# C-H-Chien/Trifocal_Pose_Estimation_using_Improved_GPUHC

Measured on NVIDIA B200. Metric: RANSAC hypotheses/s (312 HC paths each), higher is better.
Workload: dtype c64

## Files before the change

trifocal_pose_estimation_using_improved_gpuhc_b200/codegen/gen_eval.py:

```python
#!/usr/bin/env python3
import os
import sys

import numpy as np

HERE = os.path.dirname(os.path.abspath(__file__))
PKG = os.path.dirname(HERE)
sys.path.insert(0, os.path.dirname(PKG))

N = 30
P_PAD = 33
X_PAD = 30
WARP = 32
SPEC = dict(name="trifocal_2op1p_30x30", n_vars=30, n_params=33, n_tracks=312, hx_terms=8, hx_parts=5, ht_terms=16, ht_parts=6,
            n_depths=8, trifocal=1)


def configure(spec):
    global N, P_PAD, X_PAD, SPEC
    SPEC = dict(spec)
    N, P_PAD, X_PAD = SPEC["n_vars"], SPEC["n_params"], SPEC["n_vars"]
    assert 1 <= N <= 31 and SPEC["hx_parts"] == 5 and SPEC["ht_parts"] == 6


def read_problem_dir(path):
    cfg = {}
    for line in open(os.path.join(path, "gpuhc_settings.yaml")):
        line = line.split("#")[0]
        if ":" in line:
            k, v = line.split(":", 1)
            cfg[k.strip()] = v.strip().strip('"')
    spec = dict(name=cfg["problem_name"], n_vars=int(cfg["Num_Of_Vars"]), n_params=int(cfg["Num_Of_Params"]), n_tracks=int(cfg["Num_Of_Tracks"]),
                hx_terms=int(cfg["dHdx_Max_Terms"]), hx_parts=int(cfg["dHdx_Max_Parts"]), ht_terms=int(cfg["dHdt_Max_Terms"]),
                ht_parts=int(cfg["dHdt_Max_Parts"]), n_depths=int(cfg.get("Num_Of_Depth_Vars", 0)), trifocal=int(cfg["problem_name"] == "trifocal_2op1p_30x30"))
    if spec["trifocal"]:
        spec["n_depths"] = 8
    hx = np.array(open(os.path.join(path, "dHdx_indx.txt")).read().split(), dtype=np.int64)
    ht = np.array(open(os.path.join(path, "dHdt_indx.txt")).read().split(), dtype=np.int64)
    return spec, hx, ht


_TABLES = None


def load_tables():
    if _TABLES is None:
        from trifocal_pose_estimation_using_improved_gpuhc_b200 import fixtures
        prob = fixtures.load_problem()
        hx_flat, ht_flat = prob["dHdx_indx"], prob["dHdt_indx"]
    else:
        hx_flat, ht_flat = _TABLES
    hx = np.asarray(hx_flat).reshape(N, SPEC["hx_terms"], SPEC["hx_parts"], N)
    ht = np.asarray(ht_flat).reshape(SPEC["ht_terms"], SPEC["ht_parts"], N)
    return hx, ht


def parse_terms(hx, ht):
    hx_terms = {}
    for col in range(N):
        for row in range(N):
            lst = []
            for t in range(hx.shape[1]):
                c, a, b, d, e = (int(v) for v in hx[col, t, :, row])
                if c == 0:
                    continue
                xs = [v for v in (d, e) if v != X_PAD]
                assert not (a == P_PAD and b != P_PAD)
                lst.append((c, a, b, xs))
            if lst:
                hx_terms[(row, col)] = lst
    h_terms = {}
    for row in range(N):
        lst = []
        for t in range(ht.shape[0]):
            c, a, b, d, e, f = (int(v) for v in ht[t, :, row])
            if c == 0:
                continue
            xs = [v for v in (d, e, f) if v != X_PAD]
            assert not (a == P_PAD and b != P_PAD)
            lst.append((c, a, b, xs))
        h_terms[row] = lst
    return hx_terms, h_terms


def level_schedule(hx_terms, K1, segments, seg_cols):
    P = np.zeros((N, N), bool)
    for (r, c) in hx_terms:
        P[r, c] = True
    level_of_col = {}
    groups = []
    for g, (seg, cols) in enumerate(zip(segments, seg_cols)):
        busy = {r: -1 for r in seg}
        for c in cols:
            part = [r for r in seg if P[r, c]]
            lvl = 1 + max(busy[r] for r in part)
            u = np.zeros(N, bool)
            for r in part:
                u |= P[r]
            for r in part:
                P[r] |= u
                busy[r] = lvl
            level_of_col[c] = lvl
            groups.append((lvl, g, c, part, u.copy()))
    n_levels = 1 + max([l for l, *_ in groups] or [-1])
    levels, first_shared = [], []
    for T in range(n_levels):
        here = [(g, c, part) for (l, g, c, part, u) in groups if l == T]
        for g in range(len(segments)):
            rows = [r for (gg, c, part) in here if gg == g for r in part]
            assert len(rows) == len(set(rows))
        need = np.zeros(N, bool)
        for (l, g, c, part, u) in groups:
            if l == T:
                need |= u
        shared = [c for c in range(K1, N) if need[c]]
        levels.append(here)
        first_shared.append(min(shared) if shared else N)
    return levels, level_of_col, first_shared


def column_classes(hx_terms):
    rows_of = {c: {r for (r, cc) in hx_terms if cc == c} for c in range(N)}
    order = sorted(range(N), key=lambda c: (-max((len(hx_terms[(r, c)]) for r in rows_of[c]), default=0), c))
    classes = []
    for c in order:
        if not rows_of[c]:
            continue
        for cl in classes:
            if all(not (rows_of[c] & rows_of[o]) for o in cl):
                cl.append(c)
                break
        else:
            classes.append([c])
    return [sorted(cl) for cl in classes]


def schedule(seqs):
    n = max(len(q) for q in seqs)
    return [[q[k] if k < len(q) else None for q in seqs] for k in range(n)]


def analyze_blocks(hx_terms):
    try:
        return _analyze_blocks(hx_terms)
    except AssertionError:
        return 0, [], []


def _analyze_blocks(hx_terms):
    P = np.zeros((N, N), bool)
    for (r, c) in hx_terms:
        P[r, c] = True
    parent = list(range(N))

    def find(a):
        while parent[a] != a:
            parent[a] = parent[parent[a]]
            a = parent[a]
        return a

    cand_of = []
    K1 = N
    for k in range(N):
        cand = [r for r in range(N) if P[r, k]]
        if len(cand) > 6:
            K1 = k
            break
        cand_of.append(cand)
        u = np.zeros(N, bool)
        for r in cand:
            u |= P[r]
        u[:k + 1] = False
        for r in cand:
            P[r] |= u
        for r in cand[1:]:
            parent[find(r)] = find(cand[0])
    comps = {}
    for r in range(N):
        comps.setdefault(find(r), []).append(r)
    assert K1 > 0 and all(len(rows) <= 6 for rows in comps.values())
    comps = sorted(comps.values(), key=lambda rows: min([k for k in range(K1) if set(cand_of[k]) & set(rows)] or [N]))
    segments = []
    for rows in comps:
        for seg in segments:
            if len(seg) + len(rows) <= 6 and len(seg) < 6 and len(rows) < 6:
                seg.extend(rows)
                break
        else:
            segments.append(list(rows))
    segments = [sorted(seg) for seg in segments]
    assert all(len(seg) <= 6 for seg in segments) and len(segments) * 6 <= WARP and sum(len(x) for x in segments) == N
    seg_cols = []
    for seg in segments:
        cols = [k for k in range(K1) if set(cand_of[k]) <= set(seg) and cand_of[k]]
        seg_cols.append(cols)
    assert sorted(c for cols in seg_cols for c in cols) == list(range(K1))
    for g, seg in enumerate(segments):
        for r in seg:
            for c in range(K1):
                assert (not P[r, c]) or c in seg_cols[g], (r, c)
    return K1, segments, seg_cols


def optimise_layout(n_pos, movable_sets, groups, seed=1):
    import random
    rnd = random.Random(seed)
    pos = list(range(n_pos))
    member = {}
    for gi, grp in enumerate(groups):
        for e in grp:
            member.setdefault(e, []).append(gi)

    def gcost(gi):
        cnt = {}
        for e in groups[gi]:
            k = pos[e] % 16
            cnt[k] = cnt.get(k, 0) + 1
        return max(cnt.values())

    cost = [gcost(gi) for gi in range(len(groups))]
    for mv in movable_sets:
        mv = list(mv)
        for sweep in range(8):
            improved = False
            rnd.shuffle(mv)
            for i in range(len(mv)):
                for j in range(i + 1, len(mv)):
                    e, f = mv[i], mv[j]
                    affected = set(member.get(e, [])) | set(member.get(f, []))
                    if not affected:
                        continue
                    before = sum(cost[gi] for gi in affected)
                    pos[e], pos[f] = pos[f], pos[e]
                    after = {gi: gcost(gi) for gi in affected}
                    if sum(after.values()) < before:
                        for gi, c in after.items():
                            cost[gi] = c
                        improved = True
                    else:
                        pos[e], pos[f] = pos[f], pos[e]
            if not improved:
                break
    return pos, sum(cost)


def _groups(slot_rows, field, pad_entry):
    out = []
    for row in slot_rows:
        for half in (range(0, 16), range(16, 32)):
            out.append({pad_entry if row[l] is None else row[l][field] for l in half})
    return out


def build():
    hx, ht = load_tables()
    hx_terms, h_terms = parse_terms(hx, ht)

    cq_keys = set()
    for lst in hx_terms.values():
        cq_keys.update((c, a, b) for c, a, b, _ in lst)
    for lst in h_terms.values():
        cq_keys.update((c, a, b) for c, a, b, _ in lst)
    cq_list = [(0, P_PAD, P_PAD)] + sorted(cq_keys, key=lambda k: (k[2] == P_PAD, k[1], k[2], k[0]))
    cq_index = {k: i for i, k in enumerate(cq_list)}
    dq_keys = set()
    for lst in h_terms.values():
        dq_keys.update((c, a, b) for c, a, b, _ in lst if not (a == P_PAD and b == P_PAD))
    dq_list = [(0, P_PAD, P_PAD)] + sorted(dq_keys, key=lambda k: (k[2] == P_PAD, k[1], k[2], k[0]))
    dq_index = {k: i for i, k in enumerate(dq_list)}

    K1, segments, seg_cols = analyze_blocks(hx_terms)
    levels, level_of_col, sp_first_shared = level_schedule(hx_terms, K1, segments, seg_cols)
    if len(levels) > 4 or (len(levels) + N - K1) % 2:
        K1, segments, seg_cols = 0, [], []
        levels, level_of_col, sp_first_shared = level_schedule(hx_terms, K1, segments, seg_cols)
    SEG = 6
    row_of_lane = [-1] * WARP
    for g, seg in enumerate(segments):
        for i, r in enumerate(seg):
            row_of_lane[g * SEG + i] = r
    if not segments:
        for r in range(N):
            row_of_lane[r] = r
    lane_of_row = [row_of_lane.index(r) for r in range(N)]
    nsp = len(levels)
    nd = N - K1
    col_at = [[None] * nsp for _ in range(WARP)]
    grp_mask = [[0] * nsp for _ in range(WARP)]
    grp_sub = [[0] * nsp for _ in range(WARP)]
    max_sub = 1
    for T, here in enumerate(levels):
        n_in_seg = {}
        for (g, c, part) in here:
            sub = n_in_seg.get(g, 0)
            n_in_seg[g] = sub + 1
            max_sub = max(max_sub, sub + 1)
            mask = 0
            for r in part:
                mask |= 1 << (lane_of_row[r] - g * SEG)
            for r in part:
                ln = lane_of_row[r]
                col_at[ln][T], grp_mask[ln][T], grp_sub[ln][T] = c, mask, sub
    assert max_sub <= 2

    def slot_of(lane, col):
        if col >= K1:
            return nsp + (col - K1)
        assert col_at[lane][level_of_col[col]] == col
        return level_of_col[col]

    pairs, triples = set(), set()
    for lst in list(hx_terms.values()) + list(h_terms.values()):
        for c, a, b, xs in lst:
            if len(xs) == 2:
                pairs.add(tuple(xs))
            elif len(xs) == 3:
                triples.add(tuple(xs))
    pairs, triples = sorted(pairs), sorted(triples)
    XP_PAIR0 = 32
    XP_TRI0 = XP_PAIR0 + ((len(pairs) + WARP - 1) // WARP) * WARP
    XP_TOTAL = XP_TRI0 + ((len(triples) + 7) // 8) * 8

    def xp_index(xs):
        if len(xs) == 0:
            return X_PAD
        if len(xs) == 1:
            return xs[0]
        if len(xs) == 2:
            return XP_PAIR0 + pairs.index(tuple(xs))
        return XP_TRI0 + triples.index(tuple(xs))

    classes = column_classes(hx_terms)
    col_class = {c: ci for ci, cl in enumerate(classes) for c in cl}
    hx_slots = []
    for ci, cl in enumerate(classes):
        seqs = []
        for lane in range(WARP):
            seq = []
            row = row_of_lane[lane]
            if row >= 0:
                cols = [c for c in cl if (row, c) in hx_terms]
                assert len(cols) <= 1
                if cols:
                    for c, a, b, xs in hx_terms[(row, cols[0])]:
                        seq.append((cq_index[(c, a, b)], xp_index(xs)))
            seqs.append(seq)
        for row in schedule(seqs):
            hx_slots.append((ci, row))

    def sched_rows(terms_of_row, index, drop_const):
        seqs = []
        for lane in range(WARP):
            seq = []
            if row_of_lane[lane] >= 0:
                for c, a, b, xs in terms_of_row[row_of_lane[lane]]:
                    if drop_const and a == P_PAD and b == P_PAD:
                        continue
                    seq.append((index[(c, a, b)], xp_index(xs)))
            seqs.append(seq)
        return schedule(seqs)

    h_slots = sched_rows(h_terms, cq_index, False)
    ht_slots = sched_rows(h_terms, dq_index, True)
    while len(ht_slots) < len(h_slots):
        ht_slots.append([None] * WARP)
    assert (nsp + nd) % 2 == 0, "the kernel moves register slots in pairs: levels + dense columns must be even"
    assert all(row_of_lane[l] >= 0 for l in range(N)) and all(row_of_lane[l] < 0 for l in range(N, WARP)), "rows must occupy lanes 0..N-1"
    assert all(-2 <= c <= 5 for lst in list(hx_terms.values()) + list(h_terms.values()) for c, _, _, _ in lst), "coefficients are packed into 3 bits"

    hx_rows = [row for _, row in hx_slots]
    cost0 = [sum(max(sum(1 for e in grp if e % 16 == k) for k in range(16)) for grp in _groups(r, f, pe))
             for r, f, pe in ((hx_rows + h_slots, 0, 0), (ht_slots, 0, 0), (hx_rows + h_slots + ht_slots, 1, X_PAD))]
    cq_pos, c_cq = optimise_layout(len(cq_list), [range(1, len(cq_list))], _groups(hx_rows + h_slots, 0, 0))
    dq_pos, c_dq = optimise_layout(len(dq_list), [range(1, len(dq_list))], _groups(ht_slots, 0, 0))
    xp_pos, c_xp = optimise_layout(XP_TOTAL, [range(XP_PAIR0, XP_TRI0), range(XP_TRI0, XP_TOTAL)],
                                   _groups(hx_rows + h_slots + ht_slots, 1, X_PAD))
    layout_cost = dict(before=cost0, after=[c_cq, c_dq, c_xp])

    def remap(rows, cpos):
        return [[None if p is None else (cpos[p[0]], xp_pos[p[1]]) for p in row] for row in rows]

    hx_slots = [(ci, r) for (ci, _), r in zip(hx_slots, remap(hx_rows, cq_pos))]
    h_slots = remap(h_slots, cq_pos)
    ht_slots = remap(ht_slots, dq_pos)
    cq_by_pos = [(0, P_PAD, P_PAD)] * len(cq_list)
    for e, q in enumerate(cq_pos):
        cq_by_pos[q] = cq_list[e]
    dq_by_pos = [(0, P_PAD, P_PAD)] * len(dq_list)
    for e, q in enumerate(dq_pos):
        dq_by_pos[q] = dq_list[e]
    cq_list, dq_list = cq_by_pos, dq_by_pos
    pair_by_pos = [None] * (XP_TRI0 - XP_PAIR0)
    for i, pr in enumerate(pairs):
        pair_by_pos[xp_pos[XP_PAIR0 + i] - XP_PAIR0] = pr
    tri_by_pos = [None] * (XP_TOTAL - XP_TRI0)
    for i, tr in enumerate(triples):
        tri_by_pos[xp_pos[XP_TRI0 + i] - XP_TRI0] = tr

    nslot = nsp + nd
    scatter = []
    sel_of_lane = [0] * WARP
    nz_of_lane = [0] * WARP
    n_sel = 0
    for t in range(nslot):
        cls_per_lane = []
        for lane in range(WARP):
            col = col_at[lane][t] if t < nsp else (K1 + (t - nsp) if row_of_lane[lane] >= 0 else None)
            cls_per_lane.append(col_class.get(col) if col is not None else None)
        used = sorted({c for c in cls_per_lane if c is not None})
        assert 1 <= len(used) <= 2
        if len(used) == 1:
            scatter.append((used[0], -1, -1))
        else:
            scatter.append((used[0], used[1], n_sel))
            for lane in range(WARP):
                if cls_per_lane[lane] == used[1]:
                    sel_of_lane[lane] |= 1 << n_sel
            n_sel += 1
    for lane in range(WARP):
        row = row_of_lane[lane]
        if row < 0:
            continue
        for c in range(N):
            if (row, c) in hx_terms:
                nz_of_lane[lane] |= 1 << slot_of(lane, c)
    return dict(hx_terms=hx_terms, h_terms=h_terms, cq_list=cq_list, dq_list=dq_list, classes=classes,
                col_class=col_class, hx_slots=hx_slots, h_slots=h_slots, ht_slots=ht_slots,
                K1=K1, segments=segments, seg_cols=seg_cols, row_of_lane=row_of_lane, lane_of_row=lane_of_row,
                nsp=nsp, nd=nd, nslot=nslot, sp_first_shared=sp_first_shared, levels=levels, level_of_col=level_of_col,
                col_at=col_at, grp_mask=grp_mask, grp_sub=grp_sub, max_sub=max_sub, scatter=scatter, sel_of_lane=sel_of_lane, nz_of_lane=nz_of_lane, n_sel=n_sel,
                pairs=pair_by_pos, triples=tri_by_pos, XP_PAIR0=XP_PAIR0, XP_TRI0=XP_TRI0, XP_TOTAL=XP_TOTAL,
                layout_cost=layout_cost)


def pack_word(payload):
    idx, xp = (0, X_PAD) if payload is None else payload
    return (idx * 8) | ((xp * 8) << 16)


def pack_xp_word(xs):
    xs = list(xs) + [X_PAD] * (3 - len(xs))
    return (xs[0] * 8) | ((xs[1] * 8) << 8) | ((xs[2] * 8) << 16)


def pack_build_word(key):
    c, a, b = key
    return (a * 8) | ((b * 8) << 9) | ((c + 2) << 18)


def emit(g, path):
    ncq, ndq = len(g["cq_list"]), len(g["dq_list"])
    rounds = lambda n: (n + WARP - 1) // WARP
    L = []
    w = L.append
    w("// GENERATED by codegen/gen_eval.py from the problem's evaluation-index tables — do not edit.")
    w("// Problem: %s (%d equations, %d unknowns, %d parameters, %d paths)." % (SPEC["name"], N, N, SPEC["n_params"], SPEC["n_tracks"]))
    w("#ifndef HC_PROBLEM_GEN_H")
    w("#define HC_PROBLEM_GEN_H")
    w("#define HCG_N %d" % N)
    w("#define HCG_NUM_PARAMS %d" % SPEC["n_params"])
    w("#define HCG_NUM_CQ %d   /* coef*p_a*p_b table (entry 0 == 0) */" % ncq)
    w("#define HCG_NUM_DQ %d   /* coef*(dp_a*p_b + dp_b*p_a) table (entry 0 == 0) */" % ndq)
    w("#define HCG_CQ_ROUNDS %d" % rounds(ncq))
    w("#define HCG_DQ_ROUNDS %d" % rounds(ndq))
    w("#define HCG_NUM_CLASSES %d" % len(g["classes"]))
    w("#define HCG_HX_SLOTS %d" % len(g["hx_slots"]))
    w("#define HCG_H_SLOTS %d" % len(g["h_slots"]))
    w("#define HCG_HT_SLOTS %d" % len(g["ht_slots"]))
    nnz = len(g["hx_terms"])
    nterms = sum(len(v) for v in g["hx_terms"].values())
    w("#define HCG_HX_NNZ %d" % nnz)
    w("#define HCG_HX_TERMS %d" % nterms)
    w("#define HCG_H_TERMS %d" % sum(len(v) for v in g["h_terms"].values()))
    off_cq = 0
    off_dq = off_cq + rounds(ncq)
    off_pair = off_dq + rounds(ndq)
    off_tri = off_pair + rounds(len(g["pairs"]))
    off_hx = off_tri + rounds(len(g["triples"]))
    w("#define HCG_XP_PAIR0 %d   /* x-product array: [0,32) x itself, then %d pairs, then %d triples */" % (g["XP_PAIR0"], len(g["pairs"]), len(g["triples"])))
    w("#define HCG_XP_TRI0 %d" % g["XP_TRI0"])
    w("#define HCG_XP_TOTAL %d" % g["XP_TOTAL"])
    w("#define HCG_NUM_PAIRS %d" % len(g["pairs"]))
    w("#define HCG_NUM_TRIPLES %d" % len(g["triples"]))
    w("#define HCG_PAIR_ROUNDS %d" % rounds(len(g["pairs"])))
    w("#define HCG_TRI_ROUNDS %d" % rounds(len(g["triples"])))
    w("#define HCG_TBL_PAIR %d" % off_pair)
    w("#define HCG_TBL_TRI %d" % off_tri)
    off_h = off_hx + len(g["hx_slots"])
    off_ht = off_h + len(g["h_slots"])
    total = off_ht + len(g["ht_slots"])
    w("#define HCG_TBL_CQ %d" % off_cq)
    w("#define HCG_TBL_DQ %d" % off_dq)
    w("#define HCG_TBL_HX %d" % off_hx)
    w("#define HCG_TBL_H %d" % off_h)
    w("#define HCG_TBL_HT %d" % off_ht)
    w("#define HCG_TBL_ROWS %d" % total)
    rows = []
    for lst, n in ((g["cq_list"], ncq), (g["dq_list"], ndq)):
        for r in range(rounds(n)):
            rows.append([pack_build_word(lst[r * WARP + l]) if r * WARP + l < n else pack_build_word((0, P_PAD, P_PAD))
                         for l in range(WARP)])
    for lst in (g["pairs"], g["triples"]):
        for r in range(rounds(len(lst))):
            rows.append([pack_xp_word(lst[r * WARP + l]) if r * WARP + l < len(lst) and lst[r * WARP + l] is not None else pack_xp_word([])
                         for l in range(WARP)])
    for _, row in g["hx_slots"]:
        rows.append([pack_word(p) for p in row])
    for row in g["h_slots"]:
        rows.append([pack_word(p) for p in row])
    for row in g["ht_slots"]:
        rows.append([pack_word(p) for p in row])
    assert len(rows) == total
    w("// packed per-lane operand words, [row][lane]")
    w("#define HCG_TBL_INIT { \\")
    for r in rows:
        w("  " + ",".join("0x%08xu" % v for v in r) + ", \\")
    w("}")
    w("// block structure: %d segments of 6 lanes; sparse pivot columns per segment %s; dense columns %d..%d"
      % (len(g["segments"]), g["seg_cols"], g["K1"], N - 1))
    for T, here in enumerate(g["levels"]):
        w("//   level %d: %s" % (T, "  ".join("col %d rows %s" % (c, part) for (_, c, part) in here)))
    w("#define HCG_K1 %d        /* first dense pivot column */" % g["K1"])
    w("#define HCG_NSP %d        /* sparse slots == levels (super-steps) */" % g["nsp"])
    w("#define HCG_ND %d        /* dense slots */" % g["nd"])
    w("#define HCG_NSLOT %d     /* register slots per row */" % g["nslot"])
    w("#define HCG_SEG 6")
    w("#define HCG_NSEG %d" % max(1, len(g["segments"])))
    w("// per super-step: first register slot of the shared columns that can be non-zero in a participating row")
    w("#define HCG_SP_FIRST_SHARED_SLOT_INIT { " + ",".join([str(g["nsp"] + c - g["K1"]) for c in g["sp_first_shared"]] or ["0"]) + " }")
    w("#define HCG_ROW_OF_LANE_INIT { " + ",".join(str(r) for r in g["row_of_lane"]) + " }")
    w("#define HCG_LANE_OF_ROW_INIT { " + ",".join(str(r) for r in g["lane_of_row"]) + " }")
    info, cols, grps = [], [], []
    for lane in range(WARP):
        assert g["nslot"] <= 20 and g["n_sel"] <= 4 and g["nsp"] <= 4
        info.append(g["nz_of_lane"][lane] | (g["sel_of_lane"][lane] << 20))
        packed, gp = 0, 0
        for t in range(g["nsp"]):
            if g["col_at"][lane][t] is not None:
                packed |= g["col_at"][lane][t] << (5 * t)
                gp |= (g["grp_mask"][lane][t] | (g["grp_sub"][lane][t] << 6)) << (7 * t)
        cols.append(packed)
        grps.append(gp)
    w("#define HCG_LANEINFO_INIT { " + ",".join("0x%08xu" % v for v in info) + " }")
    w("#define HCG_LANECOLS_INIT { " + ",".join("0x%08xu" % v for v in cols) + " }   /* 5 bits per level: the private column the lane's row meets there */")
    w("#define HCG_LANEGRP_INIT { " + ",".join("0x%08xu" % v for v in grps) + " }   /* 7 bits per level: lanes of my pivot group (6, relative to the segment) | group index << 6; 0 = idle */")
    w("#define HCG_MAX_GROUPS_PER_SEG %d" % g["max_sub"])
    w("// X(slot, class): one Hx term slot; acc[class] += cq * xprod")
    begs, prev = [], None
    for i, (ci, _) in enumerate(g["hx_slots"]):
        if ci != prev:
            assert prev is None or ci == prev + 1
            begs.append(i)
            prev = ci
    begs.append(len(g["hx_slots"]))
    assert len(begs) == len(g["classes"]) + 1
    w("#define HCG_HX_CLASS_BEGIN_INIT { " + ",".join(str(b) for b in begs) + " }   /* first Hx slot of every class, then the end */")
    w("#define HCG_HX_SLOT_LIST(X) \\")
    for s, (ci, _) in enumerate(g["hx_slots"]):
        w("  X(%d, %d) \\" % (s, ci))
    w("")
    w("// X(slot, classA, classB, selbit): A[slot] = lane has a non-zero there ? acc[selbit set ? classB : classA] : 0")
    w("#define HCG_HX_SCATTER_LIST(X) \\")
    for t, (ca, cb, sb) in enumerate(g["scatter"]):
        w("  X(%d, %d, %d, %d) \\" % (t, ca, cb, sb))
    w("")
    w("// problem identity: the kernel takes every size from this header (codegen/gen_eval.py --problem-dir compiles another problem)")
    w("#define HCG_PROBLEM_NAME \"%s\"" % SPEC["name"])
    w("#define HCG_TRACKS %d        /* homotopy paths per hypothesis (Num_Of_Tracks) */" % SPEC["n_tracks"])
    w("#define HCG_NUM_DEPTHS %d      /* leading variables that are depths: positive-depth pruning tests them (0: no pruning) */" % SPEC["n_depths"])
    w("#define HCG_TRIFOCAL %d        /* 1: the trifocal relative-pose problem (in-kernel scoring, pose records, target-parameter gather) */" % SPEC["trifocal"])
    w("")
    w("#endif")
    text = "\n".join(L) + "\n"
    with open(path, "w") as f:
        f.write(text)
    return text


def compile_problem(problem_dir, out):
    global _TABLES
    spec, hx, ht = read_problem_dir(problem_dir)
    configure(spec)
    _TABLES = (hx, ht)
    g = build()
    emit(g, out)
    return g


def main():
    import argparse
    ap = argparse.ArgumentParser(description=__doc__.split("\n")[0])
    ap.add_argument("--problem-dir", default=None, help="problems/<name>/ in the reference's layout (default: the packaged trifocal_2op1p_30x30 tables)")
    ap.add_argument("--out", default=None, help="header to write (default: csrc/hc_problem_gen.h, or csrc/hc_problem_gen_<name>.h with --problem-dir)")
    a = ap.parse_args()
    if a.problem_dir:
        spec = read_problem_dir(a.problem_dir)[0]
        out = a.out or os.path.join(PKG, "csrc", "hc_problem_gen_%s.h" % spec["name"])
        g = compile_problem(a.problem_dir, out)
        print("problem %s: N %d, parameters %d, paths %d | K1 %d segments %s | classes %s | Hx slots %d, H slots %d, Ht slots %d | cq %d dq %d | pairs %d triples %d"
              % (SPEC["name"], N, SPEC["n_params"], SPEC["n_tracks"], g["K1"], g["segments"], g["classes"], len(g["hx_slots"]), len(g["h_slots"]),
                 len(g["ht_slots"]), len(g["cq_list"]), len(g["dq_list"]), sum(p is not None for p in g["pairs"]), sum(t is not None for t in g["triples"])))
        print("wrote", out)
        return
    g = build()
    out = a.out or os.path.join(PKG, "csrc", "hc_problem_gen.h")
    emit(g, out)
    print("classes:", g["classes"])
    print("K1 %d segments %s seg_cols %s" % (g["K1"], g["segments"], g["seg_cols"]))
    print("row_of_lane", g["row_of_lane"])
    print("scatter", g["scatter"])
    print("cq entries %d, dq entries %d" % (len(g["cq_list"]), len(g["dq_list"])))
    print("Hx slots %d (ref 240), H slots %d (ref 16), Ht slots %d (ref 16)" %
          (len(g["hx_slots"]), len(g["h_slots"]), len(g["ht_slots"])))
    print("gather wavefront model (cq, dq, xp) before/after layout optimisation:", g["layout_cost"])
    print("hx_slots", [(ci, sum(p is not None for p in row)) for ci, row in g["hx_slots"]])
    print("h_slots", [sum(p is not None for p in row) for row in g["h_slots"]])
    print("ht_slots", [sum(p is not None for p in row) for row in g["ht_slots"]])
    print("wrote", out)


if __name__ == "__main__":
    main()
```

trifocal_pose_estimation_using_improved_gpuhc_b200/csrc/hc_problem_gen.h:

```cpp
#ifndef HC_PROBLEM_GEN_H
#define HC_PROBLEM_GEN_H
#define HCG_N 30
#define HCG_NUM_PARAMS 33
#define HCG_NUM_CQ 93
#define HCG_NUM_DQ 89
#define HCG_CQ_ROUNDS 3
#define HCG_DQ_ROUNDS 3
#define HCG_NUM_CLASSES 6
#define HCG_HX_SLOTS 25
#define HCG_H_SLOTS 16
#define HCG_HT_SLOTS 16
#define HCG_HX_NNZ 170
#define HCG_HX_TERMS 558
#define HCG_H_TERMS 360
#define HCG_XP_PAIR0 32
#define HCG_XP_TRI0 96
#define HCG_XP_TOTAL 144
#define HCG_NUM_PAIRS 64
#define HCG_NUM_TRIPLES 48
#define HCG_PAIR_ROUNDS 2
#define HCG_TRI_ROUNDS 2
#define HCG_TBL_PAIR 6
#define HCG_TBL_TRI 8
#define HCG_TBL_CQ 0
#define HCG_TBL_DQ 3
#define HCG_TBL_HX 10
#define HCG_TBL_H 35
#define HCG_TBL_HT 51
#define HCG_TBL_ROWS 67
#define HCG_TBL_INIT { \
  0x000a1108u,0x0001e000u,0x000e1068u,0x00021060u,0x0011e000u,0x00121098u,0x001210c8u,0x000df000u,0x0011f000u,0x0001e008u,0x00121108u,0x000210f8u,0x0011e008u,0x0001f008u,0x0005f008u,0x000df008u,0x000e10e8u,0x00061068u,0x00060030u,0x000e0030u,0x000e1108u,0x00020038u,0x00060038u,0x00021030u,0x00120038u,0x000e1010u,0x000e1018u,0x000e1020u,0x000e1028u,0x000610c8u,0x00061030u,0x000e1030u, \
  0x00121030u,0x000e10d8u,0x001210c0u,0x000e1038u,0x00121038u,0x000e1040u,0x000e1048u,0x000e1050u,0x000e1058u,0x0011f008u,0x00061060u,0x000e1060u,0x00121060u,0x00021068u,0x000e10c8u,0x000e1080u,0x00121068u,0x000e1070u,0x000e1078u,0x00021100u,0x000e10b8u,0x000e0038u,0x00061090u,0x000e1090u,0x00121090u,0x00021098u,0x0001f000u,0x000e1098u,0x00061108u,0x000e10a0u,0x000e10a8u,0x000e10b0u, \
  0x0005f000u,0x00120030u,0x000610c0u,0x000e10c0u,0x00061038u,0x0005e008u,0x000de000u,0x00021090u,0x000610f0u,0x000e10d0u,0x00021038u,0x000e10e0u,0x000210c0u,0x000210f0u,0x00020030u,0x000e10f0u,0x0005e000u,0x000de008u,0x000610f8u,0x000e10f8u,0x001210f8u,0x001210f0u,0x00061100u,0x000e1100u,0x00121100u,0x00021108u,0x000210c8u,0x00061098u,0x000e1088u,0x000a1108u,0x000a1108u,0x000a1108u, \
  0x000a1108u,0x0001e000u,0x0005e000u,0x000de000u,0x0011e000u,0x00060038u,0x0005f000u,0x000df000u,0x0011f000u,0x0001e008u,0x0005e008u,0x000de008u,0x0011e008u,0x0001f008u,0x0005f008u,0x000df008u,0x00061068u,0x0011f008u,0x00060030u,0x000e0030u,0x000e10c8u,0x00020038u,0x00021090u,0x000e0038u,0x00120038u,0x000e1010u,0x000e1018u,0x000e1020u,0x000e1028u,0x00021030u,0x00061030u,0x000e1030u, \
  0x00121030u,0x00021038u,0x00061038u,0x000e1038u,0x00121038u,0x000e1040u,0x000e1048u,0x000e1050u,0x000e1058u,0x00021060u,0x00061060u,0x000e1060u,0x00121060u,0x00021068u,0x00020030u,0x000e1068u,0x00121068u,0x000e1070u,0x000e1078u,0x000e1080u,0x000e1088u,0x00120030u,0x00061090u,0x000e1090u,0x00121090u,0x00021098u,0x00061098u,0x000e1098u,0x00121098u,0x000e10a0u,0x000e10a8u,0x000e10b0u, \
  0x000e10b8u,0x000210c0u,0x000610c0u,0x000e10c0u,0x00061100u,0x000210c8u,0x000610c8u,0x0001f000u,0x001210c8u,0x000e10d0u,0x000e10d8u,0x000e10e0u,0x000e10e8u,0x000210f0u,0x000610f0u,0x000e10f0u,0x001210f0u,0x000210f8u,0x000610f8u,0x000e10f8u,0x001210f8u,0x00021100u,0x001210c0u,0x000e1100u,0x00121100u,0x000a1108u,0x000a1108u,0x000a1108u,0x000a1108u,0x000a1108u,0x000a1108u,0x000a1108u, \
  0x00f0f0f0u,0x00f0f0f0u,0x00f0d000u,0x00f0d800u,0x00f0e000u,0x00f0d808u,0x00f0c008u,0x00f0c808u,0x00f0c078u,0x00f0c860u,0x00f0e008u,0x00f0e808u,0x00f0d008u,0x00f0f0f0u,0x00f0f0f0u,0x00f0d860u,0x00f0f0f0u,0x00f0e860u,0x00f0d060u,0x00f0c878u,0x00f0d078u,0x00f0d878u,0x00f0c060u,0x00f0e878u,0x00f0c0c0u,0x00f0c8c0u,0x00f0d0c0u,0x00f0f0f0u,0x00f0d0c8u,0x00f0d0d0u,0x00f0f0f0u,0x00f0e0d8u, \
  0x00f0e8d8u,0x00f0d8d8u,0x00f0e8e0u,0x00f0e8e8u,0x00f0f0f0u,0x00f0f0f0u,0x00f0e0e0u,0x00f0f0f0u,0x00f0f0f0u,0x00f0e800u,0x00f0f0f0u,0x00f0f0f0u,0x00f0f0f0u,0x00f0c800u,0x00f0f0f0u,0x00f0c000u,0x00f0f0f0u,0x00f0f0f0u,0x00f0f0f0u,0x00f0f0f0u,0x00f0c8c8u,0x00f0f0f0u,0x00f0f0f0u,0x00f0f0f0u,0x00f0f0f0u,0x00f0f0f0u,0x00f0f0f0u,0x00f0e078u,0x00f0e060u,0x00f0f0f0u,0x00f0f0f0u,0x00f0f0f0u, \
  0x00c0c000u,0x00c8c000u,0x00d0c000u,0x00c8c800u,0x00d0c800u,0x00d0d000u,0x00e8e078u,0x00e0d800u,0x00e8d800u,0x00e0e000u,0x00e8e000u,0x00e8e060u,0x00c0c008u,0x00c8c008u,0x00d0c008u,0x00c8c808u,0x00d0c808u,0x00d0d008u,0x00d8d808u,0x00e0d808u,0x00e8d808u,0x00d0c060u,0x00e8e008u,0x00e8e808u,0x00c0c060u,0x00c8c060u,0x00d8d800u,0x00c8c860u,0x00d0c860u,0x00d0d060u,0x00d8d860u,0x00e0d860u, \
  0x00e8d860u,0x00e0e060u,0x00e8e800u,0x00e8e860u,0x00c0c078u,0x00c8c078u,0x00d0c078u,0x00c8c878u,0x00d0c878u,0x00d0d078u,0x00d8d878u,0x00e0d878u,0x00e8d878u,0x00e0e078u,0x00e0e008u,0x00e8e878u,0x00f0f0f0u,0x00f0f0f0u,0x00f0f0f0u,0x00f0f0f0u,0x00f0f0f0u,0x00f0f0f0u,0x00f0f0f0u,0x00f0f0f0u,0x00f0f0f0u,0x00f0f0f0u,0x00f0f0f0u,0x00f0f0f0u,0x00f0f0f0u,0x00f0f0f0u,0x00f0f0f0u,0x00f0f0f0u, \
  0x00d00120u,0x00c00050u,0x00c80100u,0x00e80120u,0x00d80050u,0x00e00100u,0x00d00180u,0x00c00050u,0x00c80160u,0x00e80180u,0x00d80050u,0x00e00160u,0x00f000c8u,0x00f000d0u,0x00f000a0u,0x00f000d8u,0x00f000e0u,0x00f000a0u,0x00d00028u,0x01c001d8u,0x00c801c0u,0x00e80028u,0x020801d8u,0x00e001c0u,0x00d00030u,0x01c00170u,0x00c80110u,0x00e80030u,0x02080170u,0x00e00110u,0x00f00000u,0x00f00000u, \
  0x00c802c8u,0x00f00220u,0x00c00250u,0x00e002c8u,0x00f00220u,0x00d80250u,0x00c802c8u,0x00f00088u,0x00c00168u,0x00e002c8u,0x00f00088u,0x00d80168u,0x00f00000u,0x00f00000u,0x00f00000u,0x00f00000u,0x00f00000u,0x00f00000u,0x00f001b0u,0x00d00238u,0x00c001c8u,0x00f001b0u,0x00e80238u,0x00d801c8u,0x00f00210u,0x00d00260u,0x00c002d0u,0x00f00210u,0x00e80260u,0x00d802d0u,0x00f00000u,0x00f00000u, \
  0x00f000f0u,0x00d000b8u,0x01c000a0u,0x00f000f0u,0x00e800b8u,0x020800a0u,0x00f00150u,0x00d00018u,0x01c000a0u,0x00f00150u,0x00e80018u,0x020800a0u,0x00f00000u,0x00f00000u,0x00f00000u,0x00f00000u,0x00f00000u,0x00f00000u,0x01c001b0u,0x00f002d8u,0x01d00238u,0x020801b0u,0x00f002d8u,0x02000238u,0x01c00210u,0x00f000e8u,0x01d00260u,0x02080210u,0x00f000e8u,0x02000260u,0x00f00000u,0x00f00000u, \
  0x01d002c8u,0x01e002c8u,0x02a000a0u,0x020002c8u,0x021002c8u,0x023000a0u,0x01d002c8u,0x01e002c8u,0x02a000a0u,0x020002c8u,0x021002c8u,0x023000a0u,0x00f00000u,0x00f00000u,0x00f00000u,0x00f00000u,0x00f00000u,0x00f00000u,0x02a001b8u,0x02a002d8u,0x01e001c8u,0x023001b8u,0x023002d8u,0x021001c8u,0x02a00218u,0x02a000e8u,0x01e002d0u,0x02300218u,0x023000e8u,0x021002d0u,0x00f00000u,0x00f00000u, \
  0x01c000f0u,0x01c00118u,0x01e801e0u,0x020800f0u,0x02080118u,0x021801e0u,0x01c00150u,0x01c00010u,0x01e801e0u,0x02080150u,0x02080010u,0x021801e0u,0x00f00000u,0x00f00000u,0x00f00000u,0x00f00000u,0x00f00000u,0x00f00000u,0x01e801b8u,0x01e801d8u,0x00f00000u,0x021801b8u,0x021801d8u,0x00f00000u,0x01e80218u,0x01e80170u,0x00f00000u,0x02180218u,0x02180170u,0x00f00000u,0x00f00000u,0x00f00000u, \
  0x02a000f8u,0x02a00220u,0x01d000b8u,0x023000f8u,0x02300220u,0x020000b8u,0x02a00158u,0x02a00088u,0x01d00018u,0x02300158u,0x02300088u,0x02000018u,0x00f00000u,0x00f00000u,0x00f00000u,0x00f00000u,0x00f00000u,0x00f00000u,0x01c801c8u,0x01c80238u,0x00f00000u,0x01f801c8u,0x01f80238u,0x00f00000u,0x01c802d0u,0x01c80260u,0x00f00000u,0x01f802d0u,0x01f80260u,0x00f00000u,0x00f00000u,0x00f00000u, \
  0x01e800f8u,0x01e80118u,0x01e00250u,0x021800f8u,0x02180118u,0x02100250u,0x01e80158u,0x01e80010u,0x01e00168u,0x02180158u,0x02180010u,0x02100168u,0x00f00000u,0x00f00000u,0x00f00000u,0x00f00000u,0x00f00000u,0x00f00000u,0x00f00000u,0x00f00000u,0x00f00000u,0x00f00000u,0x00f00000u,0x00f00000u,0x00f00000u,0x00f00000u,0x00f00000u,0x00f00000u,0x00f00000u,0x00f00000u,0x00f00000u,0x00f00000u, \
  0x01c80250u,0x01c800b8u,0x00f001e0u,0x01f80250u,0x01f800b8u,0x00f001e0u,0x01c80168u,0x01c80018u,0x00f001e0u,0x01f80168u,0x01f80018u,0x00f001e0u,0x00f00000u,0x00f00000u,0x00f00000u,0x00f00000u,0x00f00000u,0x00f00000u,0x00f00000u,0x00f00000u,0x00f00000u,0x00f00000u,0x00f00000u,0x00f00000u,0x00f00000u,0x00f00000u,0x00f00000u,0x00f00000u,0x00f00000u,0x00f00000u,0x00f00000u,0x00f00000u, \
  0x011002c8u,0x00000050u,0x02780050u,0x024802c8u,0x00000050u,0x01180050u,0x016002c8u,0x00080050u,0x01300050u,0x015802c8u,0x00080050u,0x01280050u,0x00d00268u,0x00f002a8u,0x00c002a8u,0x00e80268u,0x00f002a8u,0x00d802a8u,0x00d00058u,0x00f002a0u,0x00c002a0u,0x00e80058u,0x00f002a0u,0x00d802a0u,0x00d00198u,0x00f002c0u,0x00c002c0u,0x00e80198u,0x00f002c0u,0x00d802c0u,0x00f00000u,0x00f00000u, \
  0x027800b8u,0x026800b8u,0x00000250u,0x011800b8u,0x012000b8u,0x00000250u,0x01300018u,0x01380018u,0x00080168u,0x01280018u,0x01500018u,0x00080168u,0x00c00008u,0x00c80008u,0x00f00048u,0x00d80008u,0x00e00008u,0x00f00048u,0x00c001d0u,0x00c801d0u,0x006001c8u,0x00d801d0u,0x00e001d0u,0x006001c8u,0x00c00270u,0x00c80270u,0x007802d0u,0x00d80270u,0x00e00270u,0x007802d0u,0x00f00000u,0x00f00000u, \
  0x02680250u,0x02780120u,0x011000b8u,0x01200250u,0x01180120u,0x024800b8u,0x01380168u,0x01300180u,0x01600018u,0x01500168u,0x01280180u,0x01580018u,0x00c80048u,0x00c00060u,0x00d00008u,0x00e00048u,0x00d80060u,0x00e80008u,0x00c80068u,0x00c00148u,0x00f00068u,0x00e00068u,0x00d80148u,0x00f00068u,0x00c800a8u,0x00c000c0u,0x00f000a8u,0x00e000a8u,0x00d800c0u,0x00f000a8u,0x00f00000u,0x00f00000u, \
  0x00f00000u,0x00f00000u,0x00f00000u,0x00f00000u,0x00f00000u,0x00f00000u,0x00f00000u,0x00f00000u,0x00f00000u,0x00f00000u,0x00f00000u,0x00f00000u,0x00f00000u,0x00f00000u,0x00f00000u,0x00f00000u,0x00f00000u,0x00f00000u,0x01b00238u,0x01480238u,0x00d001d0u,0x01780238u,0x02e00238u,0x00e801d0u,0x01400260u,0x01980260u,0x00d00270u,0x01a80260u,0x02d80260u,0x00e80270u,0x00f00000u,0x00f00000u, \
  0x00f00000u,0x00f00000u,0x00f00000u,0x00f00000u,0x00f00000u,0x00f00000u,0x00f00000u,0x00f00000u,0x00f00000u,0x00f00000u,0x00f00000u,0x00f00000u,0x00f00000u,0x00f00000u,0x00f00000u,0x00f00000u,0x00f00000u,0x00f00000u,0x014801c8u,0x01b00028u,0x01900238u,0x02e001c8u,0x01780028u,0x01880238u,0x019802d0u,0x01400030u,0x01a00260u,0x02d802d0u,0x01a80030u,0x01b80260u,0x00f00000u,0x00f00000u, \
  0x02680100u,0x011002c8u,0x00000100u,0x01200100u,0x024802c8u,0x00000100u,0x01380160u,0x016002c8u,0x00080160u,0x01500160u,0x015802c8u,0x00080160u,0x00c80020u,0x00d00268u,0x00f00020u,0x00e00020u,0x00e80268u,0x00f00020u,0x00c80040u,0x00d00058u,0x00f00040u,0x00e00040u,0x00e80058u,0x00f00040u,0x00c80208u,0x00d00198u,0x00f00208u,0x00e00208u,0x00e80198u,0x00f00208u,0x00f00000u,0x00f00000u, \
  0x000002c8u,0x027800b8u,0x02680050u,0x000002c8u,0x011800b8u,0x01200050u,0x000802c8u,0x01300018u,0x01380050u,0x000802c8u,0x01280018u,0x01500050u,0x00f00268u,0x00c00008u,0x00c802a8u,0x00f00268u,0x00d80008u,0x00e002a8u,0x00f00058u,0x00c001d0u,0x006001c0u,0x00f00058u,0x00d801d0u,0x006001c0u,0x00f00198u,0x00c00270u,0x00780110u,0x00f00198u,0x00d80270u,0x00780110u,0x00f00000u,0x00f00000u, \
  0x02780250u,0x02680250u,0x01100250u,0x01180250u,0x01200250u,0x02480250u,0x01300168u,0x01380168u,0x01600168u,0x01280168u,0x01500168u,0x01580168u,0x00c00048u,0x00c80048u,0x00d00048u,0x00d80048u,0x00e00048u,0x00e80048u,0x00c00068u,0x00c80068u,0x00c802a0u,0x00d80068u,0x00e00068u,0x00e002a0u,0x00c000a8u,0x00c800a8u,0x00c802c0u,0x00d800a8u,0x00e000a8u,0x00e002c0u,0x00f00000u,0x00f00000u, \
  0x00f00000u,0x00f00000u,0x00f00000u,0x00f00000u,0x00f00000u,0x00f00000u,0x00f00000u,0x00f00000u,0x00f00000u,0x00f00000u,0x00f00000u,0x00f00000u,0x00f00000u,0x00f00000u,0x00f00000u,0x00f00000u,0x00f00000u,0x00f00000u,0x014801c0u,0x01b00238u,0x00d00068u,0x02e001c0u,0x01780238u,0x00e80068u,0x01980110u,0x01400260u,0x00d000a8u,0x02d80110u,0x01a80260u,0x00e800a8u,0x00f00000u,0x00f00000u, \
  0x00f00000u,0x00f00000u,0x00f00000u,0x00f00000u,0x00f00000u,0x00f00000u,0x00f00000u,0x00f00000u,0x00f00000u,0x00f00000u,0x00f00000u,0x00f00000u,0x00f00000u,0x00f00000u,0x00f00000u,0x00f00000u,0x00f00000u,0x00f00000u,0x01b001c8u,0x014801c8u,0x019001c8u,0x017801c8u,0x02e001c8u,0x018801c8u,0x014002d0u,0x019802d0u,0x01a002d0u,0x01a802d0u,0x02d802d0u,0x01b802d0u,0x00f00000u,0x00f00000u, \
  0x00000120u,0x01100120u,0x011002c8u,0x00000120u,0x02480120u,0x024802c8u,0x00080180u,0x01600180u,0x016002c8u,0x00080180u,0x01580180u,0x015802c8u,0x00f00060u,0x00d00060u,0x00d00268u,0x00f00060u,0x00e80060u,0x00e80268u,0x00f00148u,0x00d00148u,0x00d00058u,0x00f00148u,0x00e80148u,0x00e80058u,0x00f000c0u,0x00d000c0u,0x00d00198u,0x00f000c0u,0x00e800c0u,0x00e80198u,0x00f00000u,0x00f00000u, \
  0x027802c8u,0x026802c8u,0x027800b8u,0x011802c8u,0x012002c8u,0x011800b8u,0x013002c8u,0x013802c8u,0x01300018u,0x012802c8u,0x015002c8u,0x01280018u,0x00c00268u,0x00c80268u,0x00c00008u,0x00d80268u,0x00e00268u,0x00d80008u,0x00600028u,0x00600238u,0x00c001d0u,0x00600028u,0x00600238u,0x00d801d0u,0x00780030u,0x00780260u,0x00c00270u,0x00780030u,0x00780260u,0x00d80270u,0x00f00000u,0x00f00000u, \
  0x01100100u,0x000000b8u,0x02680250u,0x02480100u,0x000000b8u,0x01200250u,0x01600160u,0x00080018u,0x01380168u,0x01580160u,0x00080018u,0x01500168u,0x00d00020u,0x00f00008u,0x00c80048u,0x00e80020u,0x00f00008u,0x00e00048u,0x00c00058u,0x00c80058u,0x00c80068u,0x00d80058u,0x00e00058u,0x00e00068u,0x00c00198u,0x00c80198u,0x00c800a8u,0x00d80198u,0x00e00198u,0x00e000a8u,0x00f00000u,0x00f00000u, \
  0x00f00000u,0x00f00000u,0x00f00000u,0x00f00000u,0x00f00000u,0x00f00000u,0x00f00000u,0x00f00000u,0x00f00000u,0x00f00000u,0x00f00000u,0x00f00000u,0x00f00000u,0x00f00000u,0x00f00000u,0x00f00000u,0x00f00000u,0x00f00000u,0x00d00040u,0x00f001d0u,0x01b00238u,0x00e80040u,0x00f001d0u,0x01780238u,0x00d00208u,0x00f00270u,0x01400260u,0x00e80208u,0x00f00270u,0x01a80260u,0x00f00000u,0x00f00000u, \
  0x00f00000u,0x00f00000u,0x00f00000u,0x00f00000u,0x00f00000u,0x00f00000u,0x00f00000u,0x00f00000u,0x00f00000u,0x00f00000u,0x00f00000u,0x00f00000u,0x00f00000u,0x00f00000u,0x00f00000u,0x00f00000u,0x00f00000u,0x00f00000u,0x019001c0u,0x01900028u,0x014801c8u,0x018801c0u,0x01880028u,0x02e001c8u,0x01a00110u,0x01a00030u,0x019802d0u,0x01b80110u,0x01b80030u,0x02d802d0u,0x00f00000u,0x00f00000u, \
  0x00f00128u,0x00f00130u,0x00f000a0u,0x00f00138u,0x00f00140u,0x00f000a0u,0x00f00188u,0x00f00190u,0x00f000a0u,0x00f00178u,0x00f002e0u,0x00f000a0u,0x00f00000u,0x00f00000u,0x00f00000u,0x00f00000u,0x00f00000u,0x00f00000u,0x00f000c8u,0x00f000d0u,0x00f000a0u,0x00f000d8u,0x00f000e0u,0x00f000a0u,0x00f00128u,0x00f00130u,0x00f000a0u,0x00f00138u,0x00f00140u,0x00f000a0u,0x00f00000u,0x00f00000u, \
  0x00f001e0u,0x00f001e0u,0x00f001e0u,0x00f001e0u,0x00f001e0u,0x00f001e0u,0x00f001e0u,0x00f001e0u,0x00f001e0u,0x00f001e0u,0x00f001e0u,0x00f001e0u,0x00f001e0u,0x00f001e0u,0x00f001e0u,0x00f001e0u,0x00f001e0u,0x00f001e0u,0x00f001e8u,0x00f001f0u,0x00f00000u,0x00f001f8u,0x00f001a0u,0x00f00000u,0x00f00248u,0x00f00108u,0x00f00000u,0x00f00258u,0x00f00080u,0x00f00000u,0x00f00000u,0x00f00000u, \
  0x00180128u,0x00180130u,0x001800a0u,0x00300138u,0x00300140u,0x003000a0u,0x00200188u,0x00200190u,0x002000a0u,0x00380178u,0x003802e0u,0x003800a0u,0x001000c8u,0x001000d0u,0x001000a0u,0x002800d8u,0x002800e0u,0x002800a0u,0x004000c8u,0x004000d0u,0x004000a0u,0x004800d8u,0x004800e0u,0x004800a0u,0x00500128u,0x00500130u,0x005000a0u,0x00580138u,0x00580140u,0x005800a0u,0x00f00000u,0x00f00000u, \
  0x000000f0u,0x00000220u,0x000001e0u,0x000000f0u,0x00000220u,0x000001e0u,0x00080150u,0x00080088u,0x000801e0u,0x00080150u,0x00080088u,0x000801e0u,0x00f00280u,0x00f00228u,0x00f00240u,0x00f00280u,0x00f00228u,0x00f00240u,0x00f00200u,0x00f00070u,0x00f00290u,0x00f00200u,0x00f00070u,0x00f00290u,0x00f00090u,0x00f000b0u,0x00f002b0u,0x00f00090u,0x00f000b0u,0x00f002b0u,0x00f00000u,0x00f00000u, \
  0x009001e0u,0x009801e0u,0x00a001e0u,0x00a801e0u,0x00b001e0u,0x00b801e0u,0x009001e0u,0x009801e0u,0x00a001e0u,0x00a801e0u,0x00b001e0u,0x00b801e0u,0x009001e0u,0x009801e0u,0x00a001e0u,0x00a801e0u,0x00b001e0u,0x00b801e0u,0x006001b0u,0x006002d8u,0x01c00298u,0x006001b0u,0x006002d8u,0x02080298u,0x00780210u,0x007800e8u,0x01c002b8u,0x00780210u,0x007800e8u,0x020802b8u,0x00f00000u,0x00f00000u, \
  0x026802c8u,0x02780050u,0x030000a0u,0x012002c8u,0x01180050u,0x03d000a0u,0x013802c8u,0x01300050u,0x036000a0u,0x015002c8u,0x01280050u,0x039000a0u,0x00c80268u,0x00c002a8u,0x01c00278u,0x00e00268u,0x00d802a8u,0x02080278u,0x006801e8u,0x006801f0u,0x02a00298u,0x007001f8u,0x007001a0u,0x02300298u,0x00800248u,0x00800108u,0x02a002b8u,0x00880258u,0x00880080u,0x023002b8u,0x00f00000u,0x00f00000u, \
  0x030000f0u,0x03000118u,0x031800a0u,0x03d000f0u,0x03d00118u,0x034800a0u,0x03600150u,0x03600010u,0x037800a0u,0x03900150u,0x03900010u,0x047000a0u,0x01c00280u,0x01c00288u,0x02a00278u,0x02080280u,0x02080288u,0x02300278u,0x00c80058u,0x00c002a0u,0x01e80290u,0x00e00058u,0x00d802a0u,0x02180290u,0x00c80198u,0x00c002c0u,0x01e802b0u,0x00e00198u,0x00d802c0u,0x021802b0u,0x00f00000u,0x00f00000u, \
  0x031800f8u,0x03180220u,0x032801e0u,0x034800f8u,0x03480220u,0x041001e0u,0x03780158u,0x03780088u,0x038801e0u,0x04700158u,0x04700088u,0x03b801e0u,0x02a00230u,0x02a00228u,0x01e80240u,0x02300230u,0x02300228u,0x02180240u,0x01c00200u,0x01c00078u,0x00c80040u,0x02080200u,0x02080078u,0x00e00040u,0x01c00090u,0x01c001a8u,0x00c80208u,0x02080090u,0x020801a8u,0x00e00208u,0x00f00000u,0x00f00000u, \
  0x032800f8u,0x03280118u,0x02680100u,0x041000f8u,0x04100118u,0x01200100u,0x03880158u,0x03880010u,0x01380160u,0x03b80158u,0x03b80010u,0x01500160u,0x01e80230u,0x01e80288u,0x00c80020u,0x02180230u,0x02180288u,0x00e00020u,0x02a00038u,0x02a00070u,0x00c00068u,0x02300038u,0x02300070u,0x00d80068u,0x02a00098u,0x02a000b0u,0x00c000a8u,0x02300098u,0x023000b0u,0x00d800a8u,0x00f00000u,0x00f00000u, \
  0x01100120u,0x011000b8u,0x02780250u,0x02480120u,0x024800b8u,0x01180250u,0x01600180u,0x01600018u,0x01300168u,0x01580180u,0x01580018u,0x01280168u,0x00d00060u,0x00d00008u,0x00c00048u,0x00e80060u,0x00e80008u,0x00d80048u,0x01e80038u,0x01e80078u,0x014801c0u,0x02180038u,0x02180078u,0x02e001c0u,0x01e80098u,0x01e801a8u,0x01980110u,0x02180098u,0x021801a8u,0x02d80110u,0x00f00000u,0x00f00000u, \
  0x031002c8u,0x032002c8u,0x031000b8u,0x034002c8u,0x035002c8u,0x034000b8u,0x037002c8u,0x038002c8u,0x03700018u,0x03a002c8u,0x03b002c8u,0x03a00018u,0x01d00268u,0x01e00268u,0x01d00008u,0x02000268u,0x02100268u,0x02000008u,0x03c001b0u,0x03c001d8u,0x01b001c8u,0x03f001b0u,0x03f001d8u,0x017801c8u,0x04200210u,0x04200170u,0x014002d0u,0x04500210u,0x04500170u,0x01a802d0u,0x00f00000u,0x00f00000u, \
  0x03080250u,0x030800b8u,0x03200250u,0x03380250u,0x033800b8u,0x03500250u,0x03680168u,0x03680018u,0x03800168u,0x03980168u,0x03980018u,0x03b00168u,0x01c80048u,0x01c80008u,0x01e00048u,0x01f80048u,0x01f80008u,0x02100048u,0x03d801b8u,0x03d802d8u,0x01d001d0u,0x040801b8u,0x040802d8u,0x020001d0u,0x04380218u,0x043800e8u,0x01d00270u,0x04680218u,0x046800e8u,0x02000270u,0x00f00000u,0x00f00000u, \
  0x00f00000u,0x00f00000u,0x00f00000u,0x00f00000u,0x00f00000u,0x00f00000u,0x00f00000u,0x00f00000u,0x00f00000u,0x00f00000u,0x00f00000u,0x00f00000u,0x00f00000u,0x00f00000u,0x00f00000u,0x00f00000u,0x00f00000u,0x00f00000u,0x03e801b8u,0x03e801d8u,0x01e00068u,0x041801b8u,0x041801d8u,0x02100068u,0x04480218u,0x04480170u,0x01e000a8u,0x04780218u,0x04780170u,0x021000a8u,0x00f00000u,0x00f00000u, \
  0x00f00000u,0x00f00000u,0x00f00000u,0x00f00000u,0x00f00000u,0x00f00000u,0x00f00000u,0x00f00000u,0x00f00000u,0x00f00000u,0x00f00000u,0x00f00000u,0x00f00000u,0x00f00000u,0x00f00000u,0x00f00000u,0x00f00000u,0x00f00000u,0x00d00148u,0x00d001d0u,0x03a80238u,0x00e80148u,0x00e801d0u,0x04000238u,0x00d000c0u,0x00d00270u,0x04300260u,0x00e800c0u,0x00e80270u,0x04600260u,0x00f00000u,0x00f00000u, \
  0x00f00000u,0x00f00000u,0x00f00000u,0x00f00000u,0x00f00000u,0x00f00000u,0x00f00000u,0x00f00000u,0x00f00000u,0x00f00000u,0x00f00000u,0x00f00000u,0x00f00000u,0x00f00000u,0x00f00000u,0x00f00000u,0x00f00000u,0x00f00000u,0x01900028u,0x01900238u,0x03e001c8u,0x01880028u,0x01880238u,0x035801c8u,0x01a00030u,0x01a00260u,0x044002d0u,0x01b80030u,0x01b80260u,0x033002d0u,0x00f00000u,0x00f00000u, \
  0x00f00000u,0x00f00000u,0x00f00000u,0x00f00000u,0x00f00000u,0x00f00000u,0x00f00000u,0x00f00000u,0x00f00000u,0x00f00000u,0x00f00000u,0x00f00000u,0x00f00000u,0x00f00000u,0x00f00000u,0x00f00000u,0x00f00000u,0x00f00000u,0x01d00058u,0x01e00058u,0x00f00000u,0x02000058u,0x02100058u,0x00f00000u,0x01d00198u,0x01e00198u,0x00f00000u,0x02000198u,0x02100198u,0x00f00000u,0x00f00000u,0x00f00000u, \
  0x00f00000u,0x00f00000u,0x00f00000u,0x00f00000u,0x00f00000u,0x00f00000u,0x00f00000u,0x00f00000u,0x00f00000u,0x00f00000u,0x00f00000u,0x00f00000u,0x00f00000u,0x00f00000u,0x00f00000u,0x00f00000u,0x00f00000u,0x00f00000u,0x01c80068u,0x01c801d0u,0x00f00000u,0x01f80068u,0x01f801d0u,0x00f00000u,0x01c800a8u,0x01c80270u,0x00f00000u,0x01f800a8u,0x01f80270u,0x00f00000u,0x00f00000u,0x00f00000u, \
  0x00f00000u,0x00f00000u,0x00f00000u,0x00f00000u,0x00f00000u,0x00f00000u,0x00f00000u,0x00f00000u,0x00f00000u,0x00f00000u,0x00f00000u,0x00f00000u,0x00f00000u,0x00f00000u,0x00f00000u,0x00f00000u,0x00f00000u,0x00f00000u,0x03c801c8u,0x03c80238u,0x00f00000u,0x03f801c8u,0x03f80238u,0x00f00000u,0x042802d0u,0x04280260u,0x00f00000u,0x045802d0u,0x04580260u,0x00f00000u,0x00f00000u,0x00f00000u, \
  0x00180128u,0x00180130u,0x02680100u,0x00300138u,0x00300140u,0x01200100u,0x00200188u,0x00200190u,0x01380160u,0x00380198u,0x003801a0u,0x01500160u,0x001000c8u,0x001000d0u,0x00f00270u,0x002800d8u,0x002800e0u,0x00f00270u,0x004000c8u,0x004000d0u,0x00f00290u,0x004800d8u,0x004800e0u,0x00f00290u,0x00500128u,0x00500130u,0x00f00220u,0x00580138u,0x00580140u,0x00f00220u,0x00f00000u,0x00f00000u, \
  0x000000f0u,0x00000110u,0x02780108u,0x000000f0u,0x00000110u,0x01180108u,0x00080150u,0x00080080u,0x01300168u,0x00080150u,0x00080080u,0x01280168u,0x00f00010u,0x00f00050u,0x01c00278u,0x00f00010u,0x00f00050u,0x02080278u,0x00f00030u,0x00f00070u,0x01c00298u,0x00f00030u,0x00f00070u,0x02080298u,0x00f00090u,0x00f00028u,0x01c002b8u,0x00f00090u,0x00f00028u,0x020802b8u,0x00f00000u,0x00f00000u, \
  0x030000f0u,0x03000118u,0x031000e8u,0x03d000f0u,0x03d00118u,0x034000e8u,0x03600150u,0x03600178u,0x03700148u,0x03900150u,0x03900178u,0x03a00148u,0x00c80268u,0x00c00280u,0x02a00278u,0x00e00268u,0x00d80280u,0x02300278u,0x006001b0u,0x006001d0u,0x02a00298u,0x006001b0u,0x006001d0u,0x02300298u,0x00780210u,0x00780230u,0x02a002b8u,0x00780210u,0x00780230u,0x023002b8u,0x00f00000u,0x00f00000u, \
  0x031800f8u,0x03180110u,0x03200108u,0x034800f8u,0x03480110u,0x03500108u,0x03780158u,0x03780080u,0x03800168u,0x04700158u,0x04700080u,0x03b00168u,0x01c00010u,0x01c00058u,0x01e80270u,0x02080010u,0x02080058u,0x02180270u,0x006801e8u,0x006801f0u,0x01e80290u,0x007001f8u,0x00700200u,0x02180290u,0x00800248u,0x00800250u,0x01e80220u,0x00880258u,0x00880260u,0x02180220u,0x00f00000u,0x00f00000u, \
  0x032800f8u,0x03280118u,0x00f00000u,0x041000f8u,0x04100118u,0x00f00000u,0x03880158u,0x03880178u,0x00f00000u,0x03b80158u,0x03b80178u,0x00f00000u,0x02a00018u,0x02a00050u,0x00c80020u,0x02300018u,0x02300050u,0x00e00020u,0x00c80288u,0x00c002a0u,0x00c80040u,0x00e00288u,0x00d802a0u,0x00e00040u,0x00c802a8u,0x00c002c0u,0x00c801a8u,0x00e002a8u,0x00d802c0u,0x00e001a8u,0x00f00000u,0x00f00000u, \
  0x01100120u,0x011000e8u,0x00f00000u,0x02480120u,0x024800e8u,0x00f00000u,0x01600180u,0x01600148u,0x00f00000u,0x01580180u,0x01580148u,0x00f00000u,0x01e80018u,0x01e80058u,0x00c00048u,0x02180018u,0x02180058u,0x00d80048u,0x01c00030u,0x01c00078u,0x00c00068u,0x02080030u,0x02080078u,0x00d80068u,0x01c00090u,0x01c000b8u,0x00c000a8u,0x02080090u,0x020800b8u,0x00d800a8u,0x00f00000u,0x00f00000u, \
  0x03080108u,0x030800e8u,0x00f00000u,0x03380108u,0x033800e8u,0x00f00000u,0x03680168u,0x03680148u,0x00f00000u,0x03980168u,0x03980148u,0x00f00000u,0x00d00060u,0x00d00008u,0x01d00008u,0x00e80060u,0x00e80008u,0x02000008u,0x02a00038u,0x02a00070u,0x014801c0u,0x02300038u,0x02300070u,0x02e001c0u,0x02a00098u,0x02a00028u,0x019802b0u,0x02300098u,0x02300028u,0x02d802b0u,0x00f00000u,0x00f00000u, \
  0x00f00000u,0x00f00000u,0x00f00000u,0x00f00000u,0x00f00000u,0x00f00000u,0x00f00000u,0x00f00000u,0x00f00000u,0x00f00000u,0x00f00000u,0x00f00000u,0x01d00268u,0x01e00268u,0x01e00048u,0x02000268u,0x02100268u,0x02100048u,0x01e80038u,0x01e80078u,0x01b001c8u,0x02180038u,0x02180078u,0x017801c8u,0x01e80098u,0x01e800b8u,0x01400228u,0x02180098u,0x021800b8u,0x01a80228u,0x00f00000u,0x00f00000u, \
  0x00f00000u,0x00f00000u,0x00f00000u,0x00f00000u,0x00f00000u,0x00f00000u,0x00f00000u,0x00f00000u,0x00f00000u,0x00f00000u,0x00f00000u,0x00f00000u,0x01c80048u,0x01c80008u,0x00f00000u,0x01f80048u,0x01f80008u,0x00f00000u,0x03c001b0u,0x03c001d8u,0x01d00238u,0x03f001b0u,0x03f001d8u,0x02000238u,0x04200210u,0x042000a0u,0x01d00170u,0x04500210u,0x045000a0u,0x02000170u,0x00f00000u,0x00f00000u, \
  0x00f00000u,0x00f00000u,0x00f00000u,0x00f00000u,0x00f00000u,0x00f00000u,0x00f00000u,0x00f00000u,0x00f00000u,0x00f00000u,0x00f00000u,0x00f00000u,0x00f00000u,0x00f00000u,0x00f00000u,0x00f00000u,0x00f00000u,0x00f00000u,0x03d801b8u,0x03d801d0u,0x01e00068u,0x040801b8u,0x040801d0u,0x02100068u,0x04380218u,0x04380230u,0x01e000a8u,0x04680218u,0x04680230u,0x021000a8u,0x00f00000u,0x00f00000u, \
  0x00f00000u,0x00f00000u,0x00f00000u,0x00f00000u,0x00f00000u,0x00f00000u,0x00f00000u,0x00f00000u,0x00f00000u,0x00f00000u,0x00f00000u,0x00f00000u,0x00f00000u,0x00f00000u,0x00f00000u,0x00f00000u,0x00f00000u,0x00f00000u,0x03e801b8u,0x03e801d8u,0x03a800b0u,0x041801b8u,0x041801d8u,0x040000b0u,0x04480218u,0x044800a0u,0x04300208u,0x04780218u,0x047800a0u,0x04600208u,0x00f00000u,0x00f00000u, \
  0x00f00000u,0x00f00000u,0x00f00000u,0x00f00000u,0x00f00000u,0x00f00000u,0x00f00000u,0x00f00000u,0x00f00000u,0x00f00000u,0x00f00000u,0x00f00000u,0x00f00000u,0x00f00000u,0x00f00000u,0x00f00000u,0x00f00000u,0x00f00000u,0x00d00088u,0x00d00238u,0x03e001c8u,0x00e80088u,0x00e80238u,0x035801c8u,0x00d000c0u,0x00d00170u,0x04400228u,0x00e800c0u,0x00e80170u,0x03300228u,0x00f00000u,0x00f00000u, \
  0x00f00000u,0x00f00000u,0x00f00000u,0x00f00000u,0x00f00000u,0x00f00000u,0x00f00000u,0x00f00000u,0x00f00000u,0x00f00000u,0x00f00000u,0x00f00000u,0x00f00000u,0x00f00000u,0x00f00000u,0x00f00000u,0x00f00000u,0x00f00000u,0x019001e0u,0x019000b0u,0x00f00000u,0x018801e0u,0x018800b0u,0x00f00000u,0x01a00240u,0x01a00208u,0x00f00000u,0x01b80240u,0x01b80208u,0x00f00000u,0x00f00000u,0x00f00000u, \
  0x00f00000u,0x00f00000u,0x00f00000u,0x00f00000u,0x00f00000u,0x00f00000u,0x00f00000u,0x00f00000u,0x00f00000u,0x00f00000u,0x00f00000u,0x00f00000u,0x00f00000u,0x00f00000u,0x00f00000u,0x00f00000u,0x00f00000u,0x00f00000u,0x01d00288u,0x01e00288u,0x00f00000u,0x02000288u,0x02100288u,0x00f00000u,0x01d002a8u,0x01e002a8u,0x00f00000u,0x020002a8u,0x021002a8u,0x00f00000u,0x00f00000u,0x00f00000u, \
  0x00f00000u,0x00f00000u,0x00f00000u,0x00f00000u,0x00f00000u,0x00f00000u,0x00f00000u,0x00f00000u,0x00f00000u,0x00f00000u,0x00f00000u,0x00f00000u,0x00f00000u,0x00f00000u,0x00f00000u,0x00f00000u,0x00f00000u,0x00f00000u,0x01c80068u,0x01c80238u,0x00f00000u,0x01f80068u,0x01f80238u,0x00f00000u,0x01c800a8u,0x01c80170u,0x00f00000u,0x01f800a8u,0x01f80170u,0x00f00000u,0x00f00000u,0x00f00000u, \
  0x00f00000u,0x00f00000u,0x00f00000u,0x00f00000u,0x00f00000u,0x00f00000u,0x00f00000u,0x00f00000u,0x00f00000u,0x00f00000u,0x00f00000u,0x00f00000u,0x00f00000u,0x00f00000u,0x00f00000u,0x00f00000u,0x00f00000u,0x00f00000u,0x03c801c8u,0x03c800b0u,0x00f00000u,0x03f801c8u,0x03f800b0u,0x00f00000u,0x04280228u,0x04280208u,0x00f00000u,0x04580228u,0x04580208u,0x00f00000u,0x00f00000u,0x00f00000u, \
}
#define HCG_K1 18
#define HCG_NSP 4
#define HCG_ND 12
#define HCG_NSLOT 16
#define HCG_SEG 6
#define HCG_NSEG 5
#define HCG_SP_FIRST_SHARED_SLOT_INIT { 4,4,4,10 }
#define HCG_ROW_OF_LANE_INIT { 3,4,5,12,13,14,6,7,8,15,16,17,0,1,2,9,10,11,18,19,20,24,25,26,21,22,23,27,28,29,-1,-1 }
#define HCG_LANE_OF_ROW_INIT { 12,13,14,0,1,2,6,7,8,15,16,17,3,4,5,9,10,11,18,19,20,24,25,26,21,22,23,27,28,29 }
#define HCG_LANEINFO_INIT { 0x00201c13u,0x00201c23u,0x00201c43u,0x0020e085u,0x0020e105u,0x0020e205u,0x00201c13u,0x00201c23u,0x00201c43u,0x0020e085u,0x0020e105u,0x0020e205u,0x00001c11u,0x00001c21u,0x00001c41u,0x0000e081u,0x0000e101u,0x0000e201u,0x00501c07u,0x00501c07u,0x00501c03u,0x0050e00bu,0x0050e00bu,0x0050e003u,0x00501c07u,0x00501c07u,0x00501c03u,0x0050e00bu,0x0050e00bu,0x0050e003u,0x00000000u,0x00000000u }
#define HCG_LANECOLS_INIT { 0x00001860u,0x00001860u,0x00001860u,0x00001860u,0x00001860u,0x00001860u,0x00001c81u,0x00001c81u,0x00001c81u,0x00001c81u,0x00001c81u,0x00001c81u,0x00000002u,0x00000002u,0x00000002u,0x00000005u,0x00000005u,0x00000005u,0x00073588u,0x00073588u,0x00073588u,0x00073589u,0x00073589u,0x00073589u,0x0008c1eau,0x0008c1eau,0x0008c1eau,0x0008c1ebu,0x0008c1ebu,0x0008c1ebu,0x00000000u,0x00000000u }
#define HCG_LANEGRP_INIT { 0x000fdfbfu,0x000fdfbfu,0x000fdfbfu,0x000fdfbfu,0x000fdfbfu,0x000fdfbfu,0x000fdfbfu,0x000fdfbfu,0x000fdfbfu,0x000fdfbfu,0x000fdfbfu,0x000fdfbfu,0x00000007u,0x00000007u,0x00000007u,0x00000078u,0x00000078u,0x00000078u,0x07efdf87u,0x07efdf87u,0x07efdf87u,0x07efdff8u,0x07efdff8u,0x07efdff8u,0x07efdf87u,0x07efdf87u,0x07efdf87u,0x07efdff8u,0x07efdff8u,0x07efdff8u,0x00000000u,0x00000000u }
#define HCG_MAX_GROUPS_PER_SEG 2
#define HCG_HX_CLASS_BEGIN_INIT { 0,8,13,18,23,24,25 }
#define HCG_HX_SLOT_LIST(X) \
  X(0, 0) \
  X(1, 0) \
  X(2, 0) \
  X(3, 0) \
  X(4, 0) \
  X(5, 0) \
  X(6, 0) \
  X(7, 0) \
  X(8, 1) \
  X(9, 1) \
  X(10, 1) \
  X(11, 1) \
  X(12, 1) \
  X(13, 2) \
  X(14, 2) \
  X(15, 2) \
  X(16, 2) \
  X(17, 2) \
  X(18, 3) \
  X(19, 3) \
  X(20, 3) \
  X(21, 3) \
  X(22, 3) \
  X(23, 4) \
  X(24, 5) \

#define HCG_HX_SCATTER_LIST(X) \
  X(0, 0, 4, 0) \
  X(1, 0, 4, 1) \
  X(2, 4, 5, 2) \
  X(3, 5, -1, -1) \
  X(4, 5, -1, -1) \
  X(5, 5, -1, -1) \
  X(6, 5, -1, -1) \
  X(7, 5, -1, -1) \
  X(8, 5, -1, -1) \
  X(9, 5, -1, -1) \
  X(10, 1, -1, -1) \
  X(11, 2, -1, -1) \
  X(12, 3, -1, -1) \
  X(13, 1, -1, -1) \
  X(14, 2, -1, -1) \
  X(15, 3, -1, -1) \

#define HCG_PROBLEM_NAME "trifocal_2op1p_30x30"
#define HCG_TRACKS 312
#define HCG_NUM_DEPTHS 8
#define HCG_TRIFOCAL 1

#endif
```

trifocal_pose_estimation_using_improved_gpuhc_b200/csrc/hc_problem_gen_coupled_quadrics_8x8.h:

```cpp
#ifndef HC_PROBLEM_GEN_H
#define HC_PROBLEM_GEN_H
#define HCG_N 8
#define HCG_NUM_PARAMS 10
#define HCG_NUM_CQ 14
#define HCG_NUM_DQ 12
#define HCG_CQ_ROUNDS 1
#define HCG_DQ_ROUNDS 1
#define HCG_NUM_CLASSES 7
#define HCG_HX_SLOTS 7
#define HCG_H_SLOTS 5
#define HCG_HT_SLOTS 5
#define HCG_HX_NNZ 38
#define HCG_HX_TERMS 38
#define HCG_H_TERMS 34
#define HCG_XP_PAIR0 32
#define HCG_XP_TRI0 64
#define HCG_XP_TOTAL 72
#define HCG_NUM_PAIRS 32
#define HCG_NUM_TRIPLES 8
#define HCG_PAIR_ROUNDS 1
#define HCG_TRI_ROUNDS 1
#define HCG_TBL_PAIR 2
#define HCG_TBL_TRI 3
#define HCG_TBL_CQ 0
#define HCG_TBL_DQ 1
#define HCG_TBL_HX 4
#define HCG_TBL_H 11
#define HCG_TBL_HT 16
#define HCG_TBL_ROWS 21
#define HCG_TBL_INIT { \
  0x0008a050u,0x00040000u,0x00041008u,0x00042010u,0x00043018u,0x00044020u,0x00045028u,0x00046030u,0x00047038u,0x000c9040u,0x000ca040u,0x000ca048u,0x000ca050u,0x0010a050u,0x0008a050u,0x0008a050u,0x0008a050u,0x0008a050u,0x0008a050u,0x0008a050u,0x0008a050u,0x0008a050u,0x0008a050u,0x0008a050u,0x0008a050u,0x0008a050u,0x0008a050u,0x0008a050u,0x0008a050u,0x0008a050u,0x0008a050u,0x0008a050u, \
  0x0008a050u,0x00040000u,0x00041008u,0x00042010u,0x00043018u,0x00044020u,0x00045028u,0x00046030u,0x00047038u,0x000c9040u,0x000ca040u,0x000ca048u,0x0008a050u,0x0008a050u,0x0008a050u,0x0008a050u,0x0008a050u,0x0008a050u,0x0008a050u,0x0008a050u,0x0008a050u,0x0008a050u,0x0008a050u,0x0008a050u,0x0008a050u,0x0008a050u,0x0008a050u,0x0008a050u,0x0008a050u,0x0008a050u,0x0008a050u,0x0008a050u, \
  0x00400000u,0x00401000u,0x00400808u,0x00404040u,0x00401008u,0x00401010u,0x00401810u,0x00402010u,0x00401818u,0x00402818u,0x00402020u,0x00403020u,0x00402828u,0x00403028u,0x00403828u,0x00400030u,0x00403030u,0x00403830u,0x00400838u,0x00403838u,0x00404040u,0x00404040u,0x00404040u,0x00404040u,0x00404040u,0x00404040u,0x00401808u,0x00404040u,0x00404040u,0x00404040u,0x00404040u,0x00404040u, \
  0x00181008u,0x00383028u,0x00404040u,0x00404040u,0x00404040u,0x00404040u,0x00404040u,0x00404040u,0x00404040u,0x00404040u,0x00404040u,0x00404040u,0x00404040u,0x00404040u,0x00404040u,0x00404040u,0x00404040u,0x00404040u,0x00404040u,0x00404040u,0x00404040u,0x00404040u,0x00404040u,0x00404040u,0x00404040u,0x00404040u,0x00404040u,0x00404040u,0x00404040u,0x00404040u,0x00404040u,0x00404040u, \
  0x00000068u,0x00100050u,0x00200068u,0x00300050u,0x00400058u,0x00100050u,0x00400058u,0x00300050u,0x00400000u,0x00400000u,0x00400000u,0x00400000u,0x00400000u,0x00400000u,0x00400000u,0x00400000u,0x00400000u,0x00400000u,0x00400000u,0x00400000u,0x00400000u,0x00400000u,0x00400000u,0x00400000u,0x00400000u,0x00400000u,0x00400000u,0x00400000u,0x00400000u,0x00400000u,0x00400000u,0x00400000u, \
  0x00180050u,0x00080068u,0x01300048u,0x00400000u,0x00380050u,0x00400058u,0x00400000u,0x00400000u,0x00400000u,0x00400000u,0x00400000u,0x00400000u,0x00400000u,0x00400000u,0x00400000u,0x00400000u,0x00400000u,0x00400000u,0x00400000u,0x00400000u,0x00400000u,0x00400000u,0x00400000u,0x00400000u,0x00400000u,0x00400000u,0x00400000u,0x00400000u,0x00400000u,0x00400000u,0x00400000u,0x00400000u, \
  0x00400058u,0x00200050u,0x01d00048u,0x00400000u,0x00400000u,0x00000050u,0x00100068u,0x00400000u,0x00400000u,0x00400000u,0x00400000u,0x00400000u,0x00400000u,0x00400000u,0x00400000u,0x00400000u,0x00400000u,0x00400000u,0x00400000u,0x00400000u,0x00400000u,0x00400000u,0x00400000u,0x00400000u,0x00400000u,0x00400000u,0x00400000u,0x00400000u,0x00400000u,0x00400000u,0x00400000u,0x00400000u, \
  0x00080050u,0x00400058u,0x01200048u,0x00400000u,0x00400000u,0x00400000u,0x00280050u,0x00180068u,0x00400000u,0x00400000u,0x00400000u,0x00400000u,0x00400000u,0x00400000u,0x00400000u,0x00400000u,0x00400000u,0x00400000u,0x00400000u,0x00400000u,0x00400000u,0x00400000u,0x00400000u,0x00400000u,0x00400000u,0x00400000u,0x00400000u,0x00400000u,0x00400000u,0x00400000u,0x00400000u,0x00400000u, \
  0x01880048u,0x00400000u,0x00380050u,0x00280068u,0x00400000u,0x00400000u,0x00180050u,0x00400058u,0x00400000u,0x00400000u,0x00400000u,0x00400000u,0x00400000u,0x00400000u,0x00400000u,0x00400000u,0x00400000u,0x00400000u,0x00400000u,0x00400000u,0x00400000u,0x00400000u,0x00400000u,0x00400000u,0x00400000u,0x00400000u,0x00400000u,0x00400000u,0x00400000u,0x00400000u,0x00400000u,0x00400000u, \
  0x01700048u,0x00400000u,0x00400058u,0x00000050u,0x00300068u,0x00400000u,0x00400000u,0x00200050u,0x00400000u,0x00400000u,0x00400000u,0x00400000u,0x00400000u,0x00400000u,0x00400000u,0x00400000u,0x00400000u,0x00400000u,0x00400000u,0x00400000u,0x00400000u,0x00400000u,0x00400000u,0x00400000u,0x00400000u,0x00400000u,0x00400000u,0x00400000u,0x00400000u,0x00400000u,0x00400000u,0x00400000u, \
  0x01680048u,0x00400000u,0x00280050u,0x00400058u,0x00080050u,0x00380068u,0x00400000u,0x00400000u,0x00400000u,0x00400000u,0x00400000u,0x00400000u,0x00400000u,0x00400000u,0x00400000u,0x00400000u,0x00400000u,0x00400000u,0x00400000u,0x00400000u,0x00400000u,0x00400000u,0x00400000u,0x00400000u,0x00400000u,0x00400000u,0x00400000u,0x00400000u,0x00400000u,0x00400000u,0x00400000u,0x00400000u, \
  0x01000060u,0x01100060u,0x01500060u,0x01600060u,0x01800060u,0x01980060u,0x01280060u,0x01400060u,0x00400000u,0x00400000u,0x00400000u,0x00400000u,0x00400000u,0x00400000u,0x00400000u,0x00400000u,0x00400000u,0x00400000u,0x00400000u,0x00400000u,0x00400000u,0x00400000u,0x00400000u,0x00400000u,0x00400000u,0x00400000u,0x00400000u,0x00400000u,0x00400000u,0x00400000u,0x00400000u,0x00400000u, \
  0x00400008u,0x00400010u,0x00400028u,0x00400030u,0x00400038u,0x00400040u,0x00400018u,0x00400020u,0x00400000u,0x00400000u,0x00400000u,0x00400000u,0x00400000u,0x00400000u,0x00400000u,0x00400000u,0x00400000u,0x00400000u,0x00400000u,0x00400000u,0x00400000u,0x00400000u,0x00400000u,0x00400000u,0x00400000u,0x00400000u,0x00400000u,0x00400000u,0x00400000u,0x00400000u,0x00400000u,0x00400000u, \
  0x01d00050u,0x01380050u,0x01700050u,0x01780050u,0x01900050u,0x01080050u,0x01480050u,0x01580050u,0x00400000u,0x00400000u,0x00400000u,0x00400000u,0x00400000u,0x00400000u,0x00400000u,0x00400000u,0x00400000u,0x00400000u,0x00400000u,0x00400000u,0x00400000u,0x00400000u,0x00400000u,0x00400000u,0x00400000u,0x00400000u,0x00400000u,0x00400000u,0x00400000u,0x00400000u,0x00400000u,0x00400000u, \
  0x00100058u,0x00180058u,0x00300058u,0x00380058u,0x00000058u,0x00080058u,0x00200058u,0x00280058u,0x00400000u,0x00400000u,0x00400000u,0x00400000u,0x00400000u,0x00400000u,0x00400000u,0x00400000u,0x00400000u,0x00400000u,0x00400000u,0x00400000u,0x00400000u,0x00400000u,0x00400000u,0x00400000u,0x00400000u,0x00400000u,0x00400000u,0x00400000u,0x00400000u,0x00400000u,0x00400000u,0x00400000u, \
  0x02080048u,0x00400000u,0x02000048u,0x00400000u,0x00400000u,0x00400000u,0x00400000u,0x00400000u,0x00400000u,0x00400000u,0x00400000u,0x00400000u,0x00400000u,0x00400000u,0x00400000u,0x00400000u,0x00400000u,0x00400000u,0x00400000u,0x00400000u,0x00400000u,0x00400000u,0x00400000u,0x00400000u,0x00400000u,0x00400000u,0x00400000u,0x00400000u,0x00400000u,0x00400000u,0x00400000u,0x00400000u, \
  0x00400008u,0x00400010u,0x00400028u,0x00400030u,0x00400038u,0x00400040u,0x00400018u,0x00400020u,0x00400000u,0x00400000u,0x00400000u,0x00400000u,0x00400000u,0x00400000u,0x00400000u,0x00400000u,0x00400000u,0x00400000u,0x00400000u,0x00400000u,0x00400000u,0x00400000u,0x00400000u,0x00400000u,0x00400000u,0x00400000u,0x00400000u,0x00400000u,0x00400000u,0x00400000u,0x00400000u,0x00400000u, \
  0x01d00050u,0x01380050u,0x01700050u,0x01780050u,0x01900050u,0x01080050u,0x01480050u,0x01580050u,0x00400000u,0x00400000u,0x00400000u,0x00400000u,0x00400000u,0x00400000u,0x00400000u,0x00400000u,0x00400000u,0x00400000u,0x00400000u,0x00400000u,0x00400000u,0x00400000u,0x00400000u,0x00400000u,0x00400000u,0x00400000u,0x00400000u,0x00400000u,0x00400000u,0x00400000u,0x00400000u,0x00400000u, \
  0x00100058u,0x00180058u,0x00300058u,0x00380058u,0x00000058u,0x00080058u,0x00200058u,0x00280058u,0x00400000u,0x00400000u,0x00400000u,0x00400000u,0x00400000u,0x00400000u,0x00400000u,0x00400000u,0x00400000u,0x00400000u,0x00400000u,0x00400000u,0x00400000u,0x00400000u,0x00400000u,0x00400000u,0x00400000u,0x00400000u,0x00400000u,0x00400000u,0x00400000u,0x00400000u,0x00400000u,0x00400000u, \
  0x02080048u,0x00400000u,0x02000048u,0x00400000u,0x00400000u,0x00400000u,0x00400000u,0x00400000u,0x00400000u,0x00400000u,0x00400000u,0x00400000u,0x00400000u,0x00400000u,0x00400000u,0x00400000u,0x00400000u,0x00400000u,0x00400000u,0x00400000u,0x00400000u,0x00400000u,0x00400000u,0x00400000u,0x00400000u,0x00400000u,0x00400000u,0x00400000u,0x00400000u,0x00400000u,0x00400000u,0x00400000u, \
  0x00400000u,0x00400000u,0x00400000u,0x00400000u,0x00400000u,0x00400000u,0x00400000u,0x00400000u,0x00400000u,0x00400000u,0x00400000u,0x00400000u,0x00400000u,0x00400000u,0x00400000u,0x00400000u,0x00400000u,0x00400000u,0x00400000u,0x00400000u,0x00400000u,0x00400000u,0x00400000u,0x00400000u,0x00400000u,0x00400000u,0x00400000u,0x00400000u,0x00400000u,0x00400000u,0x00400000u,0x00400000u, \
}
#define HCG_K1 2
#define HCG_NSP 2
#define HCG_ND 6
#define HCG_NSLOT 8
#define HCG_SEG 6
#define HCG_NSEG 2
#define HCG_SP_FIRST_SHARED_SLOT_INIT { 2,2 }
#define HCG_ROW_OF_LANE_INIT { 0,1,4,5,6,7,2,3,-1,-1,-1,-1,-1,-1,-1,-1,-1,-1,-1,-1,-1,-1,-1,-1,-1,-1,-1,-1,-1,-1,-1,-1 }
#define HCG_LANE_OF_ROW_INIT { 0,1,6,7,2,3,4,5 }
#define HCG_LANEINFO_INIT { 0x000000efu,0x0000001eu,0x000000feu,0x000000e1u,0x000000c3u,0x00000087u,0x0000003cu,0x00000078u,0x00000000u,0x00000000u,0x00000000u,0x00000000u,0x00000000u,0x00000000u,0x00000000u,0x00000000u,0x00000000u,0x00000000u,0x00000000u,0x00000000u,0x00000000u,0x00000000u,0x00000000u,0x00000000u,0x00000000u,0x00000000u,0x00000000u,0x00000000u,0x00000000u,0x00000000u,0x00000000u,0x00000000u }
#define HCG_LANECOLS_INIT { 0x00000020u,0x00000020u,0x00000020u,0x00000020u,0x00000020u,0x00000020u,0x00000000u,0x00000000u,0x00000000u,0x00000000u,0x00000000u,0x00000000u,0x00000000u,0x00000000u,0x00000000u,0x00000000u,0x00000000u,0x00000000u,0x00000000u,0x00000000u,0x00000000u,0x00000000u,0x00000000u,0x00000000u,0x00000000u,0x00000000u,0x00000000u,0x00000000u,0x00000000u,0x00000000u,0x00000000u,0x00000000u }
#define HCG_LANEGRP_INIT { 0x00001fb9u,0x00001f80u,0x00001f80u,0x00001fb9u,0x00001fb9u,0x00001fb9u,0x00000000u,0x00000000u,0x00000000u,0x00000000u,0x00000000u,0x00000000u,0x00000000u,0x00000000u,0x00000000u,0x00000000u,0x00000000u,0x00000000u,0x00000000u,0x00000000u,0x00000000u,0x00000000u,0x00000000u,0x00000000u,0x00000000u,0x00000000u,0x00000000u,0x00000000u,0x00000000u,0x00000000u,0x00000000u,0x00000000u }
#define HCG_MAX_GROUPS_PER_SEG 1
#define HCG_HX_CLASS_BEGIN_INIT { 0,1,2,3,4,5,6,7 }
#define HCG_HX_SLOT_LIST(X) \
  X(0, 0) \
  X(1, 1) \
  X(2, 2) \
  X(3, 3) \
  X(4, 4) \
  X(5, 5) \
  X(6, 6) \

#define HCG_HX_SCATTER_LIST(X) \
  X(0, 0, -1, -1) \
  X(1, 1, -1, -1) \
  X(2, 2, -1, -1) \
  X(3, 3, -1, -1) \
  X(4, 0, -1, -1) \
  X(5, 4, -1, -1) \
  X(6, 5, -1, -1) \
  X(7, 6, -1, -1) \

#define HCG_PROBLEM_NAME "coupled_quadrics_8x8"
#define HCG_TRACKS 256
#define HCG_NUM_DEPTHS 2
#define HCG_TRIFOCAL 0

#endif
```

trifocal_pose_estimation_using_improved_gpuhc_b200/csrc/hc_problem_gen_mixed_12x12.h:

```cpp
#ifndef HC_PROBLEM_GEN_H
#define HC_PROBLEM_GEN_H
#define HCG_N 12
#define HCG_NUM_PARAMS 14
#define HCG_NUM_CQ 17
#define HCG_NUM_DQ 15
#define HCG_CQ_ROUNDS 1
#define HCG_DQ_ROUNDS 1
#define HCG_NUM_CLASSES 4
#define HCG_HX_SLOTS 4
#define HCG_H_SLOTS 3
#define HCG_HT_SLOTS 3
#define HCG_HX_NNZ 36
#define HCG_HX_TERMS 36
#define HCG_H_TERMS 36
#define HCG_XP_PAIR0 32
#define HCG_XP_TRI0 64
#define HCG_XP_TOTAL 64
#define HCG_NUM_PAIRS 32
#define HCG_NUM_TRIPLES 0
#define HCG_PAIR_ROUNDS 1
#define HCG_TRI_ROUNDS 0
#define HCG_TBL_PAIR 2
#define HCG_TBL_TRI 3
#define HCG_TBL_CQ 0
#define HCG_TBL_DQ 1
#define HCG_TBL_HX 3
#define HCG_TBL_H 7
#define HCG_TBL_HT 10
#define HCG_TBL_ROWS 13
#define HCG_TBL_INIT { \
  0x0008e070u,0x00040000u,0x00041008u,0x0010e070u,0x00043018u,0x00044020u,0x00045028u,0x0004e030u,0x0004e038u,0x0004e040u,0x0004e048u,0x0004e050u,0x0004e058u,0x000ce060u,0x000ce068u,0x000ce070u,0x00042010u,0x0008e070u,0x0008e070u,0x0008e070u,0x0008e070u,0x0008e070u,0x0008e070u,0x0008e070u,0x0008e070u,0x0008e070u,0x0008e070u,0x0008e070u,0x0008e070u,0x0008e070u,0x0008e070u,0x0008e070u, \
  0x0008e070u,0x00040000u,0x00041008u,0x00042010u,0x00043018u,0x00044020u,0x00045028u,0x0004e030u,0x0004e038u,0x0004e040u,0x0004e048u,0x0004e050u,0x0004e058u,0x000ce060u,0x000ce068u,0x0008e070u,0x0008e070u,0x0008e070u,0x0008e070u,0x0008e070u,0x0008e070u,0x0008e070u,0x0008e070u,0x0008e070u,0x0008e070u,0x0008e070u,0x0008e070u,0x0008e070u,0x0008e070u,0x0008e070u,0x0008e070u,0x0008e070u, \
  0x00600000u,0x00602800u,0x00603800u,0x00600808u,0x00603008u,0x00604008u,0x00601010u,0x00603810u,0x00604810u,0x00605830u,0x00604018u,0x00605018u,0x00602020u,0x00604820u,0x00605820u,0x00602828u,0x00605028u,0x00601818u,0x00606060u,0x00606060u,0x00606060u,0x00606060u,0x00606060u,0x00606060u,0x00606060u,0x00606060u,0x00606060u,0x00606060u,0x00606060u,0x00606060u,0x00606060u,0x00606060u, \
  0x00000018u,0x00380068u,0x00100018u,0x00380070u,0x00600000u,0x00280070u,0x00480068u,0x00200018u,0x00600000u,0x00480070u,0x00600000u,0x00580070u,0x00600000u,0x00600000u,0x00600000u,0x00600000u,0x00600000u,0x00600000u,0x00600000u,0x00600000u,0x00600000u,0x00600000u,0x00600000u,0x00600000u,0x00600000u,0x00600000u,0x00600000u,0x00600000u,0x00600000u,0x00600000u,0x00600000u,0x00600000u, \
  0x00300068u,0x00080018u,0x00400068u,0x00600000u,0x00400070u,0x00000070u,0x00180018u,0x00500068u,0x00280018u,0x00600000u,0x00500070u,0x00600000u,0x00600000u,0x00600000u,0x00600000u,0x00600000u,0x00600000u,0x00600000u,0x00600000u,0x00600000u,0x00600000u,0x00600000u,0x00600000u,0x00600000u,0x00600000u,0x00600000u,0x00600000u,0x00600000u,0x00600000u,0x00600000u,0x00600000u,0x00600000u, \
  0x00080068u,0x00600000u,0x00180068u,0x00600078u,0x00080070u,0x00600000u,0x00600000u,0x00280068u,0x00580068u,0x00600078u,0x00180070u,0x00600078u,0x00600000u,0x00600000u,0x00600000u,0x00600000u,0x00600000u,0x00600000u,0x00600000u,0x00600000u,0x00600000u,0x00600000u,0x00600000u,0x00600000u,0x00600000u,0x00600000u,0x00600000u,0x00600000u,0x00600000u,0x00600000u,0x00600000u,0x00600000u, \
  0x00600000u,0x00100068u,0x00600000u,0x00000070u,0x00600078u,0x00600078u,0x00200068u,0x00600000u,0x00300068u,0x00100070u,0x00600078u,0x00200070u,0x00600000u,0x00600000u,0x00600000u,0x00600000u,0x00600000u,0x00600000u,0x00600000u,0x00600000u,0x00600000u,0x00600000u,0x00600000u,0x00600000u,0x00600000u,0x00600000u,0x00600000u,0x00600000u,0x00600000u,0x00600000u,0x00600000u,0x00600000u, \
  0x01000078u,0x01180078u,0x01300078u,0x00300078u,0x00380078u,0x00580078u,0x01880078u,0x01600078u,0x01780078u,0x00400078u,0x00480078u,0x00500078u,0x00600000u,0x00600000u,0x00600000u,0x00600000u,0x00600000u,0x00600000u,0x00600000u,0x00600000u,0x00600000u,0x00600000u,0x00600000u,0x00600000u,0x00600000u,0x00600000u,0x00600000u,0x00600000u,0x00600000u,0x00600000u,0x00600000u,0x00600000u, \
  0x00600008u,0x00600010u,0x00600080u,0x00600038u,0x00600040u,0x00600060u,0x00600020u,0x00600028u,0x00600030u,0x00600048u,0x00600050u,0x00600058u,0x00600000u,0x00600000u,0x00600000u,0x00600000u,0x00600000u,0x00600000u,0x00600000u,0x00600000u,0x00600000u,0x00600000u,0x00600000u,0x00600000u,0x00600000u,0x00600000u,0x00600000u,0x00600000u,0x00600000u,0x00600000u,0x00600000u,0x00600000u, \
  0x01200068u,0x01380068u,0x01500068u,0x01100070u,0x01280070u,0x01080070u,0x01680068u,0x01800068u,0x01480068u,0x01400070u,0x01580070u,0x01700070u,0x00600000u,0x00600000u,0x00600000u,0x00600000u,0x00600000u,0x00600000u,0x00600000u,0x00600000u,0x00600000u,0x00600000u,0x00600000u,0x00600000u,0x00600000u,0x00600000u,0x00600000u,0x00600000u,0x00600000u,0x00600000u,0x00600000u,0x00600000u, \
  0x00600008u,0x00600010u,0x00600018u,0x00600038u,0x00600040u,0x00600060u,0x00600020u,0x00600028u,0x00600030u,0x00600048u,0x00600050u,0x00600058u,0x00600000u,0x00600000u,0x00600000u,0x00600000u,0x00600000u,0x00600000u,0x00600000u,0x00600000u,0x00600000u,0x00600000u,0x00600000u,0x00600000u,0x00600000u,0x00600000u,0x00600000u,0x00600000u,0x00600000u,0x00600000u,0x00600000u,0x00600000u, \
  0x01200068u,0x01380068u,0x01500068u,0x01100070u,0x01280070u,0x01080070u,0x01680068u,0x01800068u,0x01480068u,0x01400070u,0x01580070u,0x01700070u,0x00600000u,0x00600000u,0x00600000u,0x00600000u,0x00600000u,0x00600000u,0x00600000u,0x00600000u,0x00600000u,0x00600000u,0x00600000u,0x00600000u,0x00600000u,0x00600000u,0x00600000u,0x00600000u,0x00600000u,0x00600000u,0x00600000u,0x00600000u, \
  0x00600000u,0x00600000u,0x00600000u,0x00600000u,0x00600000u,0x00600000u,0x00600000u,0x00600000u,0x00600000u,0x00600000u,0x00600000u,0x00600000u,0x00600000u,0x00600000u,0x00600000u,0x00600000u,0x00600000u,0x00600000u,0x00600000u,0x00600000u,0x00600000u,0x00600000u,0x00600000u,0x00600000u,0x00600000u,0x00600000u,0x00600000u,0x00600000u,0x00600000u,0x00600000u,0x00600000u,0x00600000u, \
}
#define HCG_K1 2
#define HCG_NSP 2
#define HCG_ND 10
#define HCG_NSLOT 12
#define HCG_SEG 6
#define HCG_NSEG 2
#define HCG_SP_FIRST_SHARED_SLOT_INIT { 5,2 }
#define HCG_ROW_OF_LANE_INIT { 0,1,2,6,7,11,3,4,5,8,9,10,-1,-1,-1,-1,-1,-1,-1,-1,-1,-1,-1,-1,-1,-1,-1,-1,-1,-1,-1,-1 }
#define HCG_LANE_OF_ROW_INIT { 0,1,2,6,7,8,3,4,9,10,11,5 }
#define HCG_LANEINFO_INIT { 0x00000043u,0x00000086u,0x0000010cu,0x000000c1u,0x00000182u,0x00000821u,0x00000218u,0x00000430u,0x00000860u,0x00000304u,0x00000608u,0x00000c10u,0x00000000u,0x00000000u,0x00000000u,0x00000000u,0x00000000u,0x00000000u,0x00000000u,0x00000000u,0x00000000u,0x00000000u,0x00000000u,0x00000000u,0x00000000u,0x00000000u,0x00000000u,0x00000000u,0x00000000u,0x00000000u,0x00000000u,0x00000000u }
#define HCG_LANECOLS_INIT { 0x00000020u,0x00000020u,0x00000000u,0x00000020u,0x00000020u,0x00000020u,0x00000000u,0x00000000u,0x00000000u,0x00000000u,0x00000000u,0x00000000u,0x00000000u,0x00000000u,0x00000000u,0x00000000u,0x00000000u,0x00000000u,0x00000000u,0x00000000u,0x00000000u,0x00000000u,0x00000000u,0x00000000u,0x00000000u,0x00000000u,0x00000000u,0x00000000u,0x00000000u,0x00000000u,0x00000000u,0x00000000u }
#define HCG_LANEGRP_INIT { 0x00001da9u,0x00001d80u,0x00000000u,0x00001da9u,0x00001d80u,0x00001da9u,0x00000000u,0x00000000u,0x00000000u,0x00000000u,0x00000000u,0x00000000u,0x00000000u,0x00000000u,0x00000000u,0x00000000u,0x00000000u,0x00000000u,0x00000000u,0x00000000u,0x00000000u,0x00000000u,0x00000000u,0x00000000u,0x00000000u,0x00000000u,0x00000000u,0x00000000u,0x00000000u,0x00000000u,0x00000000u,0x00000000u }
#define HCG_MAX_GROUPS_PER_SEG 1
#define HCG_HX_CLASS_BEGIN_INIT { 0,1,2,3,4 }
#define HCG_HX_SLOT_LIST(X) \
  X(0, 0) \
  X(1, 1) \
  X(2, 2) \
  X(3, 3) \

#define HCG_HX_SCATTER_LIST(X) \
  X(0, 0, -1, -1) \
  X(1, 1, -1, -1) \
  X(2, 0, -1, -1) \
  X(3, 1, -1, -1) \
  X(4, 0, -1, -1) \
  X(5, 1, -1, -1) \
  X(6, 2, -1, -1) \
  X(7, 3, -1, -1) \
  X(8, 2, -1, -1) \
  X(9, 3, -1, -1) \
  X(10, 2, -1, -1) \
  X(11, 3, -1, -1) \

#define HCG_PROBLEM_NAME "mixed_12x12"
#define HCG_TRACKS 64
#define HCG_NUM_DEPTHS 3
#define HCG_TRIFOCAL 0

#endif
```

Baseline: 4641.

## Replicate shared-memory table entries into padding holes to cut bank conflicts

The code generator now places duplicate copies of coefficient and x-product table entries into unused padding slots of the shared-memory tables. For each warp-half gather it uses bipartite matching to choose which copy each lane reads, lowering the maximum number of lanes that hit one bank. The per-lane read words are rewritten to point at the replicas, so the tables are larger and must be built with the replicas filled in. Build cost rises slightly and table sizes grow (XP_TOTAL 144→160).

```diff
diff --git a/trifocal_pose_estimation_using_improved_gpuhc_b200/codegen/gen_eval.py b/trifocal_pose_estimation_using_improved_gpuhc_b200/codegen/gen_eval.py
--- a/trifocal_pose_estimation_using_improved_gpuhc_b200/codegen/gen_eval.py
+++ b/trifocal_pose_estimation_using_improved_gpuhc_b200/codegen/gen_eval.py
@@ -252,6 +252,75 @@
     return out
 
 
+def _match(entries, copies, cap=1):
+    taken = {}
+
+    def augment(e, seen):
+        for q in copies[e]:
+            for j in range(cap):
+                k = (q % 16, j)
+                if k in seen:
+                    continue
+                seen.add(k)
+                if k not in taken or augment(taken[k][0], seen):
+                    taken[k] = (e, q)
+                    return True
+        return False
+
+    for e in sorted(entries):
+        augment(e, set())
+    return {e: q for e, q in taken.values()}
+
+
+def _cost(entries, copies):
+    n1 = len(_match(entries, copies))
+    cap = 1
+    while len(_match(entries, copies, cap)) < len(entries):
+        cap += 1
+    return cap, len(entries) - n1
+
+
+def place_replicas(groups, holes):
+    copies = {e: [e] for grp in groups for e in grp}
+    used = set()
+    cost = [_cost(grp, copies) for grp in groups]
+    while True:
+        short = [gi for gi, c in enumerate(cost) if c[1] > 0]
+        best = None
+        for e in sorted({e for gi in short for e in groups[gi]}):
+            by_bank = {}
+            for h in holes.get(e, ()):
+                if h not in used:
+                    by_bank.setdefault(h % 16, h)
+            for h in sorted(by_bank.values()):
+                copies[e].append(h)
+                new = {gi: _cost(groups[gi], copies) for gi in short if e in groups[gi]}
+                copies[e].pop()
+                gain = (sum(cost[gi][0] - c[0] for gi, c in new.items()), sum(cost[gi][1] - c[1] for gi, c in new.items()))
+                if gain > (0, 0) and (best is None or gain > best[0]):
+                    best = (gain, e, h, new)
+        if best is None:
+            break
+        _, e, h, new = best
+        copies[e].append(h)
+        used.add(h)
+        for gi, c in new.items():
+            cost[gi] = c
+    read = []
+    for gi, grp in enumerate(groups):
+        m = _match(grp, copies, cost[gi][0])
+        read.append(m)
+    return copies, read
+
+
+def gather_cost(rows, field, pad_entry, read=None):
+    total = 0
+    for gi, grp in enumerate(_groups(rows, field, pad_entry)):
+        pos = {read[gi].get(e, e) for e in grp} if read else grp
+        total += max(sum(1 for q in pos if q % 16 == k) for k in range(16))
+    return total
+
+
 def build():
     hx, ht = load_tables()
     hx_terms, h_terms = parse_terms(hx, ht)
@@ -397,6 +466,48 @@
     for i, tr in enumerate(triples):
         tri_by_pos[xp_pos[XP_TRI0 + i] - XP_TRI0] = tr
 
+    hx_rows = [row for _, row in hx_slots]
+    ncq, ndq = len(cq_list), len(dq_list)
+    cq_holes = list(range(ncq, (ncq + WARP - 1) // WARP * WARP))
+    dq_holes = list(range(ndq, (ndq + WARP - 1) // WARP * WARP))
+    pair_holes = [XP_PAIR0 + i for i, pr in enumerate(pair_by_pos) if pr is None]
+    tri_end = XP_TRI0 + (len(tri_by_pos) + WARP - 1) // WARP * WARP
+    tri_holes = [XP_TRI0 + i for i, tr in enumerate(tri_by_pos) if tr is None] + list(range(XP_TOTAL, tri_end))
+    cq_groups, dq_groups = _groups(hx_rows + h_slots, 0, 0), _groups(ht_slots, 0, 0)
+    xp_groups = _groups(hx_rows + h_slots + ht_slots, 1, X_PAD)
+    cq_copies, cq_read = place_replicas(cq_groups, {e: cq_holes for e in range(ncq)})
+    dq_copies, dq_read = place_replicas(dq_groups, {e: dq_holes for e in range(ndq)})
+    xp_holes = {e: pair_holes for e in range(XP_PAIR0, XP_TRI0)}
+    xp_holes.update({e: tri_holes for e in range(XP_TRI0, XP_TOTAL)})
+    xp_copies, xp_read = place_replicas(xp_groups, xp_holes)
+
+    def fill(table, base, copies, key_of, pad):
+        table = list(table)
+        for e, qs in copies.items():
+            for q in qs[1:]:
+                table.extend([pad] * (q - base + 1 - len(table)))
+                table[q - base] = key_of(e)
+        return table
+
+    cq_list = fill(cq_list, 0, cq_copies, lambda e: cq_list[e], (0, P_PAD, P_PAD))
+    dq_list = fill(dq_list, 0, dq_copies, lambda e: dq_list[e], (0, P_PAD, P_PAD))
+    xp_rep_key = lambda e: pair_by_pos[e - XP_PAIR0] if e < XP_TRI0 else tri_by_pos[e - XP_TRI0]
+    pair_by_pos = fill(pair_by_pos, XP_PAIR0, {e: qs for e, qs in xp_copies.items() if XP_PAIR0 <= e < XP_TRI0}, xp_rep_key, None)
+    tri_by_pos = fill(tri_by_pos, XP_TRI0, {e: qs for e, qs in xp_copies.items() if e >= XP_TRI0}, xp_rep_key, None)
+    assert len(pair_by_pos) == XP_TRI0 - XP_PAIR0
+    tri_by_pos += [None] * (-len(tri_by_pos) % 8)
+    XP_SIZE = XP_TRI0 + len(tri_by_pos)
+
+    def reads(rows, cread, c0, x0):
+        return [[(cread[2 * (c0 + i) + l // 16].get(p[0], p[0]), xp_read[2 * (x0 + i) + l // 16].get(p[1], p[1]))
+                 for l, p in enumerate((0, X_PAD) if p is None else p for p in row)] for i, row in enumerate(rows)]
+
+    nhx, nh = len(hx_rows), len(h_slots)
+    hx_read, h_read, ht_read = reads(hx_rows, cq_read, 0, 0), reads(h_slots, cq_read, nhx, nhx), reads(ht_slots, dq_read, 0, nhx + nh)
+    gather_model = {name: dict(floor=2 * len(rows), before=(gather_cost(rows, 0, 0), gather_cost(rows, 1, X_PAD)),
+                               after=(gather_cost(rd, 0, 0), gather_cost(rd, 1, X_PAD)))
+                    for name, rows, rd in (("Hx", hx_rows, hx_read), ("H", h_slots, h_read), ("Ht", ht_slots, ht_read))}
+
     nslot = nsp + nd
     scatter = []
     sel_of_lane = [0] * WARP
@@ -429,8 +540,9 @@
                 K1=K1, segments=segments, seg_cols=seg_cols, row_of_lane=row_of_lane, lane_of_row=lane_of_row,
                 nsp=nsp, nd=nd, nslot=nslot, sp_first_shared=sp_first_shared, levels=levels, level_of_col=level_of_col,
                 col_at=col_at, grp_mask=grp_mask, grp_sub=grp_sub, max_sub=max_sub, scatter=scatter, sel_of_lane=sel_of_lane, nz_of_lane=nz_of_lane, n_sel=n_sel,
-                pairs=pair_by_pos, triples=tri_by_pos, XP_PAIR0=XP_PAIR0, XP_TRI0=XP_TRI0, XP_TOTAL=XP_TOTAL,
-                layout_cost=layout_cost)
+                pairs=pair_by_pos, triples=tri_by_pos, XP_PAIR0=XP_PAIR0, XP_TRI0=XP_TRI0, XP_TOTAL=XP_SIZE,
+                hx_read=hx_read, h_read=h_read, ht_read=ht_read, replicas=dict(cq=cq_copies, dq=dq_copies, xp=xp_copies),
+                layout_cost=layout_cost, gather_model=gather_model)
 
 
 def pack_word(payload):
@@ -459,8 +571,8 @@
     w("#define HC_PROBLEM_GEN_H")
     w("#define HCG_N %d" % N)
     w("#define HCG_NUM_PARAMS %d" % SPEC["n_params"])
-    w("#define HCG_NUM_CQ %d   /* coef*p_a*p_b table (entry 0 == 0) */" % ncq)
-    w("#define HCG_NUM_DQ %d   /* coef*(dp_a*p_b + dp_b*p_a) table (entry 0 == 0) */" % ndq)
+    w("#define HCG_NUM_CQ %d   /* coef*p_a*p_b table (entry 0 == 0), build positions with replicas */" % ncq)
+    w("#define HCG_NUM_DQ %d   /* coef*(dp_a*p_b + dp_b*p_a) table (entry 0 == 0), build positions with replicas */" % ndq)
     w("#define HCG_CQ_ROUNDS %d" % rounds(ncq))
     w("#define HCG_DQ_ROUNDS %d" % rounds(ndq))
     w("#define HCG_NUM_CLASSES %d" % len(g["classes"]))
@@ -477,7 +589,7 @@
     off_pair = off_dq + rounds(ndq)
     off_tri = off_pair + rounds(len(g["pairs"]))
     off_hx = off_tri + rounds(len(g["triples"]))
-    w("#define HCG_XP_PAIR0 %d   /* x-product array: [0,32) x itself, then %d pairs, then %d triples */" % (g["XP_PAIR0"], len(g["pairs"]), len(g["triples"])))
+    w("#define HCG_XP_PAIR0 %d   /* x-product array: [0,32) x itself, then %d pair and %d triple build positions (replicas included) */" % (g["XP_PAIR0"], len(g["pairs"]), len(g["triples"])))
     w("#define HCG_XP_TRI0 %d" % g["XP_TRI0"])
     w("#define HCG_XP_TOTAL %d" % g["XP_TOTAL"])
     w("#define HCG_NUM_PAIRS %d" % len(g["pairs"]))
@@ -504,11 +616,7 @@
         for r in range(rounds(len(lst))):
             rows.append([pack_xp_word(lst[r * WARP + l]) if r * WARP + l < len(lst) and lst[r * WARP + l] is not None else pack_xp_word([])
                          for l in range(WARP)])
-    for _, row in g["hx_slots"]:
-        rows.append([pack_word(p) for p in row])
-    for row in g["h_slots"]:
-        rows.append([pack_word(p) for p in row])
-    for row in g["ht_slots"]:
+    for row in g["hx_read"] + g["h_read"] + g["ht_read"]:
         rows.append([pack_word(p) for p in row])
     assert len(rows) == total
     w("// packed per-lane operand words, [row][lane]")
@@ -587,6 +695,14 @@
     return g
 
 
+def print_gather_model(g):
+    print("gather wavefronts per evaluation (model / floor): coefficient table | x-product table")
+    for name, m in g["gather_model"].items():
+        print("  %-2s  permuted %d / %d | %d / %d   with replicas %d / %d | %d / %d"
+              % (name, m["before"][0], m["floor"], m["before"][1], m["floor"], m["after"][0], m["floor"], m["after"][1], m["floor"]))
+    print("  replicas: " + ", ".join("%s %d" % (t, sum(len(q) - 1 for q in c.values())) for t, c in g["replicas"].items()))
+
+
 def main():
     import argparse
     ap = argparse.ArgumentParser(description=__doc__.split("\n")[0])
@@ -600,6 +716,7 @@
         print("problem %s: N %d, parameters %d, paths %d | K1 %d segments %s | classes %s | Hx slots %d, H slots %d, Ht slots %d | cq %d dq %d | pairs %d triples %d"
               % (SPEC["name"], N, SPEC["n_params"], SPEC["n_tracks"], g["K1"], g["segments"], g["classes"], len(g["hx_slots"]), len(g["h_slots"]),
                  len(g["ht_slots"]), len(g["cq_list"]), len(g["dq_list"]), sum(p is not None for p in g["pairs"]), sum(t is not None for t in g["triples"])))
+        print_gather_model(g)
         print("wrote", out)
         return
     g = build()
@@ -613,6 +730,7 @@
     print("Hx slots %d (ref 240), H slots %d (ref 16), Ht slots %d (ref 16)" %
           (len(g["hx_slots"]), len(g["h_slots"]), len(g["ht_slots"])))
     print("gather wavefront model (cq, dq, xp) before/after layout optimisation:", g["layout_cost"])
+    print_gather_model(g)
     print("hx_slots", [(ci, sum(p is not None for p in row)) for ci, row in g["hx_slots"]])
     print("h_slots", [sum(p is not None for p in row) for row in g["h_slots"]])
     print("ht_slots", [sum(p is not None for p in row) for row in g["ht_slots"]])
diff --git a/trifocal_pose_estimation_using_improved_gpuhc_b200/csrc/hc_problem_gen.h b/trifocal_pose_estimation_using_improved_gpuhc_b200/csrc/hc_problem_gen.h
--- a/trifocal_pose_estimation_using_improved_gpuhc_b200/csrc/hc_problem_gen.h
+++ b/trifocal_pose_estimation_using_improved_gpuhc_b200/csrc/hc_problem_gen.h
@@ -2,8 +2,8 @@
 #define HC_PROBLEM_GEN_H
 #define HCG_N 30
 #define HCG_NUM_PARAMS 33
-#define HCG_NUM_CQ 93
-#define HCG_NUM_DQ 89
+#define HCG_NUM_CQ 96
+#define HCG_NUM_DQ 96
 #define HCG_CQ_ROUNDS 3
 #define HCG_DQ_ROUNDS 3
 #define HCG_NUM_CLASSES 6
@@ -15,9 +15,9 @@
 #define HCG_H_TERMS 360
 #define HCG_XP_PAIR0 32
 #define HCG_XP_TRI0 96
-#define HCG_XP_TOTAL 144
+#define HCG_XP_TOTAL 160
 #define HCG_NUM_PAIRS 64
-#define HCG_NUM_TRIPLES 48
+#define HCG_NUM_TRIPLES 64
 #define HCG_PAIR_ROUNDS 2
 #define HCG_TRI_ROUNDS 2
 #define HCG_TBL_PAIR 6
@@ -31,14 +31,14 @@
 #define HCG_TBL_INIT { \
   0x000a1108u,0x0001e000u,0x000e1068u,0x00021060u,0x0011e000u,0x00121098u,0x001210c8u,0x000df000u,0x0011f000u,0x0001e008u,0x00121108u,0x000210f8u,0x0011e008u,0x0001f008u,0x0005f008u,0x000df008u,0x000e10e8u,0x00061068u,0x00060030u,0x000e0030u,0x000e1108u,0x00020038u,0x00060038u,0x00021030u,0x00120038u,0x000e1010u,0x000e1018u,0x000e1020u,0x000e1028u,0x000610c8u,0x00061030u,0x000e1030u, \
   0x00121030u,0x000e10d8u,0x001210c0u,0x000e1038u,0x00121038u,0x000e1040u,0x000e1048u,0x000e1050u,0x000e1058u,0x0011f008u,0x00061060u,0x000e1060u,0x00121060u,0x00021068u,0x000e10c8u,0x000e1080u,0x00121068u,0x000e1070u,0x000e1078u,0x00021100u,0x000e10b8u,0x000e0038u,0x00061090u,0x000e1090u,0x00121090u,0x00021098u,0x0001f000u,0x000e1098u,0x00061108u,0x000e10a0u,0x000e10a8u,0x000e10b0u, \
-  0x0005f000u,0x00120030u,0x000610c0u,0x000e10c0u,0x00061038u,0x0005e008u,0x000de000u,0x00021090u,0x000610f0u,0x000e10d0u,0x00021038u,0x000e10e0u,0x000210c0u,0x000210f0u,0x00020030u,0x000e10f0u,0x0005e000u,0x000de008u,0x000610f8u,0x000e10f8u,0x001210f8u,0x001210f0u,0x00061100u,0x000e1100u,0x00121100u,0x00021108u,0x000210c8u,0x00061098u,0x000e1088u,0x000a1108u,0x000a1108u,0x000a1108u, \
+  0x0005f000u,0x00120030u,0x000610c0u,0x000e10c0u,0x00061038u,0x0005e008u,0x000de000u,0x00021090u,0x000610f0u,0x000e10d0u,0x00021038u,0x000e10e0u,0x000210c0u,0x000210f0u,0x00020030u,0x000e10f0u,0x0005e000u,0x000de008u,0x000610f8u,0x000e10f8u,0x001210f8u,0x001210f0u,0x00061100u,0x000e1100u,0x00121100u,0x00021108u,0x000210c8u,0x00061098u,0x000e1088u,0x000a1108u,0x0011f000u,0x0001e008u, \
   0x000a1108u,0x0001e000u,0x0005e000u,0x000de000u,0x0011e000u,0x00060038u,0x0005f000u,0x000df000u,0x0011f000u,0x0001e008u,0x0005e008u,0x000de008u,0x0011e008u,0x0001f008u,0x0005f008u,0x000df008u,0x00061068u,0x0011f008u,0x00060030u,0x000e0030u,0x000e10c8u,0x00020038u,0x00021090u,0x000e0038u,0x00120038u,0x000e1010u,0x000e1018u,0x000e1020u,0x000e1028u,0x00021030u,0x00061030u,0x000e1030u, \
   0x00121030u,0x00021038u,0x00061038u,0x000e1038u,0x00121038u,0x000e1040u,0x000e1048u,0x000e1050u,0x000e1058u,0x00021060u,0x00061060u,0x000e1060u,0x00121060u,0x00021068u,0x00020030u,0x000e1068u,0x00121068u,0x000e1070u,0x000e1078u,0x000e1080u,0x000e1088u,0x00120030u,0x00061090u,0x000e1090u,0x00121090u,0x00021098u,0x00061098u,0x000e1098u,0x00121098u,0x000e10a0u,0x000e10a8u,0x000e10b0u, \
-  0x000e10b8u,0x000210c0u,0x000610c0u,0x000e10c0u,0x00061100u,0x000210c8u,0x000610c8u,0x0001f000u,0x001210c8u,0x000e10d0u,0x000e10d8u,0x000e10e0u,0x000e10e8u,0x000210f0u,0x000610f0u,0x000e10f0u,0x001210f0u,0x000210f8u,0x000610f8u,0x000e10f8u,0x001210f8u,0x00021100u,0x001210c0u,0x000e1100u,0x00121100u,0x000a1108u,0x000a1108u,0x000a1108u,0x000a1108u,0x000a1108u,0x000a1108u,0x000a1108u, \
-  0x00f0f0f0u,0x00f0f0f0u,0x00f0d000u,0x00f0d800u,0x00f0e000u,0x00f0d808u,0x00f0c008u,0x00f0c808u,0x00f0c078u,0x00f0c860u,0x00f0e008u,0x00f0e808u,0x00f0d008u,0x00f0f0f0u,0x00f0f0f0u,0x00f0d860u,0x00f0f0f0u,0x00f0e860u,0x00f0d060u,0x00f0c878u,0x00f0d078u,0x00f0d878u,0x00f0c060u,0x00f0e878u,0x00f0c0c0u,0x00f0c8c0u,0x00f0d0c0u,0x00f0f0f0u,0x00f0d0c8u,0x00f0d0d0u,0x00f0f0f0u,0x00f0e0d8u, \
-  0x00f0e8d8u,0x00f0d8d8u,0x00f0e8e0u,0x00f0e8e8u,0x00f0f0f0u,0x00f0f0f0u,0x00f0e0e0u,0x00f0f0f0u,0x00f0f0f0u,0x00f0e800u,0x00f0f0f0u,0x00f0f0f0u,0x00f0f0f0u,0x00f0c800u,0x00f0f0f0u,0x00f0c000u,0x00f0f0f0u,0x00f0f0f0u,0x00f0f0f0u,0x00f0f0f0u,0x00f0c8c8u,0x00f0f0f0u,0x00f0f0f0u,0x00f0f0f0u,0x00f0f0f0u,0x00f0f0f0u,0x00f0f0f0u,0x00f0e078u,0x00f0e060u,0x00f0f0f0u,0x00f0f0f0u,0x00f0f0f0u, \
+  0x000e10b8u,0x000210c0u,0x000610c0u,0x000e10c0u,0x00061100u,0x000210c8u,0x000610c8u,0x0001f000u,0x001210c8u,0x000e10d0u,0x000e10d8u,0x000e10e0u,0x000e10e8u,0x000210f0u,0x000610f0u,0x000e10f0u,0x001210f0u,0x000210f8u,0x000610f8u,0x000e10f8u,0x001210f8u,0x00021100u,0x001210c0u,0x000e1100u,0x00121100u,0x00061090u,0x0001e008u,0x000df000u,0x000a1108u,0x000de000u,0x0001e000u,0x00021030u, \
+  0x00f0c0c0u,0x00f0e008u,0x00f0d000u,0x00f0d800u,0x00f0e000u,0x00f0d808u,0x00f0c008u,0x00f0c808u,0x00f0c078u,0x00f0c860u,0x00f0e008u,0x00f0e808u,0x00f0d008u,0x00f0c078u,0x00f0e800u,0x00f0d860u,0x00f0c808u,0x00f0e860u,0x00f0d060u,0x00f0c878u,0x00f0d078u,0x00f0d878u,0x00f0c060u,0x00f0e878u,0x00f0c0c0u,0x00f0c8c0u,0x00f0d0c0u,0x00f0d0c0u,0x00f0d0c8u,0x00f0d0d0u,0x00f0c0c0u,0x00f0e0d8u, \
+  0x00f0e8d8u,0x00f0d8d8u,0x00f0e8e0u,0x00f0e8e8u,0x00f0c878u,0x00f0e008u,0x00f0e0e0u,0x00f0d8d8u,0x00f0d0d0u,0x00f0e800u,0x00f0e000u,0x00f0d008u,0x00f0c800u,0x00f0c800u,0x00f0f0f0u,0x00f0c000u,0x00f0e808u,0x00f0e8d8u,0x00f0e078u,0x00f0e800u,0x00f0c8c8u,0x00f0f0f0u,0x00f0e808u,0x00f0f0f0u,0x00f0f0f0u,0x00f0f0f0u,0x00f0f0f0u,0x00f0e078u,0x00f0e060u,0x00f0f0f0u,0x00f0f0f0u,0x00f0f0f0u, \
   0x00c0c000u,0x00c8c000u,0x00d0c000u,0x00c8c800u,0x00d0c800u,0x00d0d000u,0x00e8e078u,0x00e0d800u,0x00e8d800u,0x00e0e000u,0x00e8e000u,0x00e8e060u,0x00c0c008u,0x00c8c008u,0x00d0c008u,0x00c8c808u,0x00d0c808u,0x00d0d008u,0x00d8d808u,0x00e0d808u,0x00e8d808u,0x00d0c060u,0x00e8e008u,0x00e8e808u,0x00c0c060u,0x00c8c060u,0x00d8d800u,0x00c8c860u,0x00d0c860u,0x00d0d060u,0x00d8d860u,0x00e0d860u, \
-  0x00e8d860u,0x00e0e060u,0x00e8e800u,0x00e8e860u,0x00c0c078u,0x00c8c078u,0x00d0c078u,0x00c8c878u,0x00d0c878u,0x00d0d078u,0x00d8d878u,0x00e0d878u,0x00e8d878u,0x00e0e078u,0x00e0e008u,0x00e8e878u,0x00f0f0f0u,0x00f0f0f0u,0x00f0f0f0u,0x00f0f0f0u,0x00f0f0f0u,0x00f0f0f0u,0x00f0f0f0u,0x00f0f0f0u,0x00f0f0f0u,0x00f0f0f0u,0x00f0f0f0u,0x00f0f0f0u,0x00f0f0f0u,0x00f0f0f0u,0x00f0f0f0u,0x00f0f0f0u, \
+  0x00e8d860u,0x00e0e060u,0x00e8e800u,0x00e8e860u,0x00c0c078u,0x00c8c078u,0x00d0c078u,0x00c8c878u,0x00d0c878u,0x00d0d078u,0x00d8d878u,0x00e0d878u,0x00e8d878u,0x00e0e078u,0x00e0e008u,0x00e8e878u,0x00c8c008u,0x00d8d860u,0x00f0f0f0u,0x00e8d808u,0x00f0f0f0u,0x00d0c000u,0x00e8d800u,0x00f0f0f0u,0x00f0f0f0u,0x00f0f0f0u,0x00f0f0f0u,0x00c0c008u,0x00f0f0f0u,0x00f0f0f0u,0x00f0f0f0u,0x00f0f0f0u, \
   0x00d00120u,0x00c00050u,0x00c80100u,0x00e80120u,0x00d80050u,0x00e00100u,0x00d00180u,0x00c00050u,0x00c80160u,0x00e80180u,0x00d80050u,0x00e00160u,0x00f000c8u,0x00f000d0u,0x00f000a0u,0x00f000d8u,0x00f000e0u,0x00f000a0u,0x00d00028u,0x01c001d8u,0x00c801c0u,0x00e80028u,0x020801d8u,0x00e001c0u,0x00d00030u,0x01c00170u,0x00c80110u,0x00e80030u,0x02080170u,0x00e00110u,0x00f00000u,0x00f00000u, \
   0x00c802c8u,0x00f00220u,0x00c00250u,0x00e002c8u,0x00f00220u,0x00d80250u,0x00c802c8u,0x00f00088u,0x00c00168u,0x00e002c8u,0x00f00088u,0x00d80168u,0x00f00000u,0x00f00000u,0x00f00000u,0x00f00000u,0x00f00000u,0x00f00000u,0x00f001b0u,0x00d00238u,0x00c001c8u,0x00f001b0u,0x00e80238u,0x00d801c8u,0x00f00210u,0x00d00260u,0x00c002d0u,0x00f00210u,0x00e80260u,0x00d802d0u,0x00f00000u,0x00f00000u, \
   0x00f000f0u,0x00d000b8u,0x01c000a0u,0x00f000f0u,0x00e800b8u,0x020800a0u,0x00f00150u,0x00d00018u,0x01c000a0u,0x00f00150u,0x00e80018u,0x020800a0u,0x00f00000u,0x00f00000u,0x00f00000u,0x00f00000u,0x00f00000u,0x00f00000u,0x01c001b0u,0x00f002d8u,0x01d00238u,0x020801b0u,0x00f002d8u,0x02000238u,0x01c00210u,0x00f000e8u,0x01d00260u,0x02080210u,0x00f000e8u,0x02000260u,0x00f00000u,0x00f00000u, \
@@ -49,17 +49,17 @@
   0x01c80250u,0x01c800b8u,0x00f001e0u,0x01f80250u,0x01f800b8u,0x00f001e0u,0x01c80168u,0x01c80018u,0x00f001e0u,0x01f80168u,0x01f80018u,0x00f001e0u,0x00f00000u,0x00f00000u,0x00f00000u,0x00f00000u,0x00f00000u,0x00f00000u,0x00f00000u,0x00f00000u,0x00f00000u,0x00f00000u,0x00f00000u,0x00f00000u,0x00f00000u,0x00f00000u,0x00f00000u,0x00f00000u,0x00f00000u,0x00f00000u,0x00f00000u,0x00f00000u, \
   0x011002c8u,0x00000050u,0x02780050u,0x024802c8u,0x00000050u,0x01180050u,0x016002c8u,0x00080050u,0x01300050u,0x015802c8u,0x00080050u,0x01280050u,0x00d00268u,0x00f002a8u,0x00c002a8u,0x00e80268u,0x00f002a8u,0x00d802a8u,0x00d00058u,0x00f002a0u,0x00c002a0u,0x00e80058u,0x00f002a0u,0x00d802a0u,0x00d00198u,0x00f002c0u,0x00c002c0u,0x00e80198u,0x00f002c0u,0x00d802c0u,0x00f00000u,0x00f00000u, \
   0x027800b8u,0x026800b8u,0x00000250u,0x011800b8u,0x012000b8u,0x00000250u,0x01300018u,0x01380018u,0x00080168u,0x01280018u,0x01500018u,0x00080168u,0x00c00008u,0x00c80008u,0x00f00048u,0x00d80008u,0x00e00008u,0x00f00048u,0x00c001d0u,0x00c801d0u,0x006001c8u,0x00d801d0u,0x00e001d0u,0x006001c8u,0x00c00270u,0x00c80270u,0x007802d0u,0x00d80270u,0x00e00270u,0x007802d0u,0x00f00000u,0x00f00000u, \
-  0x02680250u,0x02780120u,0x011000b8u,0x01200250u,0x01180120u,0x024800b8u,0x01380168u,0x01300180u,0x01600018u,0x01500168u,0x01280180u,0x01580018u,0x00c80048u,0x00c00060u,0x00d00008u,0x00e00048u,0x00d80060u,0x00e80008u,0x00c80068u,0x00c00148u,0x00f00068u,0x00e00068u,0x00d80148u,0x00f00068u,0x00c800a8u,0x00c000c0u,0x00f000a8u,0x00e000a8u,0x00d800c0u,0x00f000a8u,0x00f00000u,0x00f00000u, \
+  0x02680250u,0x02780120u,0x011000b8u,0x01200250u,0x01180120u,0x017000b8u,0x01380168u,0x01300180u,0x02580018u,0x01080168u,0x01280180u,0x02800018u,0x00c80048u,0x00c00060u,0x00d00008u,0x00e00048u,0x00d80060u,0x00e80008u,0x00c80068u,0x00c00148u,0x00f00068u,0x00e00068u,0x00d80148u,0x00f00068u,0x00c800a8u,0x00c000c0u,0x00f000a8u,0x00e000a8u,0x00d800c0u,0x00f000a8u,0x00f00000u,0x00f00000u, \
   0x00f00000u,0x00f00000u,0x00f00000u,0x00f00000u,0x00f00000u,0x00f00000u,0x00f00000u,0x00f00000u,0x00f00000u,0x00f00000u,0x00f00000u,0x00f00000u,0x00f00000u,0x00f00000u,0x00f00000u,0x00f00000u,0x00f00000u,0x00f00000u,0x01b00238u,0x01480238u,0x00d001d0u,0x01780238u,0x02e00238u,0x00e801d0u,0x01400260u,0x01980260u,0x00d00270u,0x01a80260u,0x02d80260u,0x00e80270u,0x00f00000u,0x00f00000u, \
   0x00f00000u,0x00f00000u,0x00f00000u,0x00f00000u,0x00f00000u,0x00f00000u,0x00f00000u,0x00f00000u,0x00f00000u,0x00f00000u,0x00f00000u,0x00f00000u,0x00f00000u,0x00f00000u,0x00f00000u,0x00f00000u,0x00f00000u,0x00f00000u,0x014801c8u,0x01b00028u,0x01900238u,0x02e001c8u,0x01780028u,0x01880238u,0x019802d0u,0x01400030u,0x01a00260u,0x02d802d0u,0x01a80030u,0x01b80260u,0x00f00000u,0x00f00000u, \
-  0x02680100u,0x011002c8u,0x00000100u,0x01200100u,0x024802c8u,0x00000100u,0x01380160u,0x016002c8u,0x00080160u,0x01500160u,0x015802c8u,0x00080160u,0x00c80020u,0x00d00268u,0x00f00020u,0x00e00020u,0x00e80268u,0x00f00020u,0x00c80040u,0x00d00058u,0x00f00040u,0x00e00040u,0x00e80058u,0x00f00040u,0x00c80208u,0x00d00198u,0x00f00208u,0x00e00208u,0x00e80198u,0x00f00208u,0x00f00000u,0x00f00000u, \
+  0x02680100u,0x011002c8u,0x00000100u,0x01200100u,0x029802c8u,0x00000100u,0x01380160u,0x025802c8u,0x00080160u,0x02280160u,0x02b002c8u,0x00080160u,0x00c80020u,0x00d00268u,0x00f00020u,0x00e00020u,0x00e80268u,0x00f00020u,0x00c80040u,0x00d00058u,0x00f00040u,0x00e00040u,0x00e80058u,0x00f00040u,0x00c80208u,0x00d00198u,0x00f00208u,0x00e00208u,0x00e80198u,0x00f00208u,0x00f00000u,0x00f00000u, \
   0x000002c8u,0x027800b8u,0x02680050u,0x000002c8u,0x011800b8u,0x01200050u,0x000802c8u,0x01300018u,0x01380050u,0x000802c8u,0x01280018u,0x01500050u,0x00f00268u,0x00c00008u,0x00c802a8u,0x00f00268u,0x00d80008u,0x00e002a8u,0x00f00058u,0x00c001d0u,0x006001c0u,0x00f00058u,0x00d801d0u,0x006001c0u,0x00f00198u,0x00c00270u,0x00780110u,0x00f00198u,0x00d80270u,0x00780110u,0x00f00000u,0x00f00000u, \
-  0x02780250u,0x02680250u,0x01100250u,0x01180250u,0x01200250u,0x02480250u,0x01300168u,0x01380168u,0x01600168u,0x01280168u,0x01500168u,0x01580168u,0x00c00048u,0x00c80048u,0x00d00048u,0x00d80048u,0x00e00048u,0x00e80048u,0x00c00068u,0x00c80068u,0x00c802a0u,0x00d80068u,0x00e00068u,0x00e002a0u,0x00c000a8u,0x00c800a8u,0x00c802c0u,0x00d800a8u,0x00e000a8u,0x00e002c0u,0x00f00000u,0x00f00000u, \
+  0x02780250u,0x02680250u,0x01100250u,0x01180250u,0x01200250u,0x01700250u,0x01300168u,0x01380168u,0x01600168u,0x01280168u,0x01080168u,0x02800168u,0x00c00048u,0x00c80048u,0x00d00048u,0x00d80048u,0x00e00048u,0x00e80048u,0x00c00068u,0x00c80068u,0x00c802a0u,0x00d80068u,0x00e00068u,0x00e002a0u,0x00c000a8u,0x00c800a8u,0x00c802c0u,0x00d800a8u,0x00e000a8u,0x00e002c0u,0x00f00000u,0x00f00000u, \
   0x00f00000u,0x00f00000u,0x00f00000u,0x00f00000u,0x00f00000u,0x00f00000u,0x00f00000u,0x00f00000u,0x00f00000u,0x00f00000u,0x00f00000u,0x00f00000u,0x00f00000u,0x00f00000u,0x00f00000u,0x00f00000u,0x00f00000u,0x00f00000u,0x014801c0u,0x01b00238u,0x00d00068u,0x02e001c0u,0x01780238u,0x00e80068u,0x01980110u,0x01400260u,0x00d000a8u,0x02d80110u,0x01a80260u,0x00e800a8u,0x00f00000u,0x00f00000u, \
   0x00f00000u,0x00f00000u,0x00f00000u,0x00f00000u,0x00f00000u,0x00f00000u,0x00f00000u,0x00f00000u,0x00f00000u,0x00f00000u,0x00f00000u,0x00f00000u,0x00f00000u,0x00f00000u,0x00f00000u,0x00f00000u,0x00f00000u,0x00f00000u,0x01b001c8u,0x014801c8u,0x019001c8u,0x017801c8u,0x02e001c8u,0x018801c8u,0x014002d0u,0x019802d0u,0x01a002d0u,0x01a802d0u,0x02d802d0u,0x01b802d0u,0x00f00000u,0x00f00000u, \
   0x00000120u,0x01100120u,0x011002c8u,0x00000120u,0x02480120u,0x024802c8u,0x00080180u,0x01600180u,0x016002c8u,0x00080180u,0x01580180u,0x015802c8u,0x00f00060u,0x00d00060u,0x00d00268u,0x00f00060u,0x00e80060u,0x00e80268u,0x00f00148u,0x00d00148u,0x00d00058u,0x00f00148u,0x00e80148u,0x00e80058u,0x00f000c0u,0x00d000c0u,0x00d00198u,0x00f000c0u,0x00e800c0u,0x00e80198u,0x00f00000u,0x00f00000u, \
   0x027802c8u,0x026802c8u,0x027800b8u,0x011802c8u,0x012002c8u,0x011800b8u,0x013002c8u,0x013802c8u,0x01300018u,0x012802c8u,0x015002c8u,0x01280018u,0x00c00268u,0x00c80268u,0x00c00008u,0x00d80268u,0x00e00268u,0x00d80008u,0x00600028u,0x00600238u,0x00c001d0u,0x00600028u,0x00600238u,0x00d801d0u,0x00780030u,0x00780260u,0x00c00270u,0x00780030u,0x00780260u,0x00d80270u,0x00f00000u,0x00f00000u, \
-  0x01100100u,0x000000b8u,0x02680250u,0x02480100u,0x000000b8u,0x01200250u,0x01600160u,0x00080018u,0x01380168u,0x01580160u,0x00080018u,0x01500168u,0x00d00020u,0x00f00008u,0x00c80048u,0x00e80020u,0x00f00008u,0x00e00048u,0x00c00058u,0x00c80058u,0x00c80068u,0x00d80058u,0x00e00058u,0x00e00068u,0x00c00198u,0x00c80198u,0x00c800a8u,0x00d80198u,0x00e00198u,0x00e000a8u,0x00f00000u,0x00f00000u, \
+  0x01100100u,0x000000b8u,0x02600250u,0x02980100u,0x000000b8u,0x01200250u,0x02580160u,0x00080018u,0x01380168u,0x02b00160u,0x00080018u,0x02280168u,0x00d00020u,0x00f00008u,0x00c80048u,0x00e80020u,0x00f00008u,0x00e00048u,0x00c00058u,0x00c80058u,0x00c80068u,0x00d80058u,0x00e00058u,0x00e00068u,0x00c00198u,0x00c80198u,0x00c800a8u,0x00d80198u,0x00e00198u,0x00e000a8u,0x00f00000u,0x00f00000u, \
   0x00f00000u,0x00f00000u,0x00f00000u,0x00f00000u,0x00f00000u,0x00f00000u,0x00f00000u,0x00f00000u,0x00f00000u,0x00f00000u,0x00f00000u,0x00f00000u,0x00f00000u,0x00f00000u,0x00f00000u,0x00f00000u,0x00f00000u,0x00f00000u,0x00d00040u,0x00f001d0u,0x01b00238u,0x00e80040u,0x00f001d0u,0x01780238u,0x00d00208u,0x00f00270u,0x01400260u,0x00e80208u,0x00f00270u,0x01a80260u,0x00f00000u,0x00f00000u, \
   0x00f00000u,0x00f00000u,0x00f00000u,0x00f00000u,0x00f00000u,0x00f00000u,0x00f00000u,0x00f00000u,0x00f00000u,0x00f00000u,0x00f00000u,0x00f00000u,0x00f00000u,0x00f00000u,0x00f00000u,0x00f00000u,0x00f00000u,0x00f00000u,0x019001c0u,0x01900028u,0x014801c8u,0x018801c0u,0x01880028u,0x02e001c8u,0x01a00110u,0x01a00030u,0x019802d0u,0x01b80110u,0x01b80030u,0x02d802d0u,0x00f00000u,0x00f00000u, \
   0x00f00128u,0x00f00130u,0x00f000a0u,0x00f00138u,0x00f00140u,0x00f000a0u,0x00f00188u,0x00f00190u,0x00f000a0u,0x00f00178u,0x00f002e0u,0x00f000a0u,0x00f00000u,0x00f00000u,0x00f00000u,0x00f00000u,0x00f00000u,0x00f00000u,0x00f000c8u,0x00f000d0u,0x00f000a0u,0x00f000d8u,0x00f000e0u,0x00f000a0u,0x00f00128u,0x00f00130u,0x00f000a0u,0x00f00138u,0x00f00140u,0x00f000a0u,0x00f00000u,0x00f00000u, \
@@ -67,12 +67,12 @@
   0x00180128u,0x00180130u,0x001800a0u,0x00300138u,0x00300140u,0x003000a0u,0x00200188u,0x00200190u,0x002000a0u,0x00380178u,0x003802e0u,0x003800a0u,0x001000c8u,0x001000d0u,0x001000a0u,0x002800d8u,0x002800e0u,0x002800a0u,0x004000c8u,0x004000d0u,0x004000a0u,0x004800d8u,0x004800e0u,0x004800a0u,0x00500128u,0x00500130u,0x005000a0u,0x00580138u,0x00580140u,0x005800a0u,0x00f00000u,0x00f00000u, \
   0x000000f0u,0x00000220u,0x000001e0u,0x000000f0u,0x00000220u,0x000001e0u,0x00080150u,0x00080088u,0x000801e0u,0x00080150u,0x00080088u,0x000801e0u,0x00f00280u,0x00f00228u,0x00f00240u,0x00f00280u,0x00f00228u,0x00f00240u,0x00f00200u,0x00f00070u,0x00f00290u,0x00f00200u,0x00f00070u,0x00f00290u,0x00f00090u,0x00f000b0u,0x00f002b0u,0x00f00090u,0x00f000b0u,0x00f002b0u,0x00f00000u,0x00f00000u, \
   0x009001e0u,0x009801e0u,0x00a001e0u,0x00a801e0u,0x00b001e0u,0x00b801e0u,0x009001e0u,0x009801e0u,0x00a001e0u,0x00a801e0u,0x00b001e0u,0x00b801e0u,0x009001e0u,0x009801e0u,0x00a001e0u,0x00a801e0u,0x00b001e0u,0x00b801e0u,0x006001b0u,0x006002d8u,0x01c00298u,0x006001b0u,0x006002d8u,0x02080298u,0x00780210u,0x007800e8u,0x01c002b8u,0x00780210u,0x007800e8u,0x020802b8u,0x00f00000u,0x00f00000u, \
-  0x026802c8u,0x02780050u,0x030000a0u,0x012002c8u,0x01180050u,0x03d000a0u,0x013802c8u,0x01300050u,0x036000a0u,0x015002c8u,0x01280050u,0x039000a0u,0x00c80268u,0x00c002a8u,0x01c00278u,0x00e00268u,0x00d802a8u,0x02080278u,0x006801e8u,0x006801f0u,0x02a00298u,0x007001f8u,0x007001a0u,0x02300298u,0x00800248u,0x00800108u,0x02a002b8u,0x00880258u,0x00880080u,0x023002b8u,0x00f00000u,0x00f00000u, \
+  0x026802c8u,0x02780050u,0x030000a0u,0x012002c8u,0x01180050u,0x03d000a0u,0x013802c8u,0x01300050u,0x04d800a0u,0x010802c8u,0x01280050u,0x039000a0u,0x00c80268u,0x00c002a8u,0x01f00278u,0x00e00268u,0x00d802a8u,0x02080278u,0x006801e8u,0x006801f0u,0x02a00298u,0x007001f8u,0x007001a0u,0x02300298u,0x00800248u,0x00800108u,0x02a002b8u,0x00880258u,0x00880080u,0x023002b8u,0x00f00000u,0x00f00000u, \
   0x030000f0u,0x03000118u,0x031800a0u,0x03d000f0u,0x03d00118u,0x034800a0u,0x03600150u,0x03600010u,0x037800a0u,0x03900150u,0x03900010u,0x047000a0u,0x01c00280u,0x01c00288u,0x02a00278u,0x02080280u,0x02080288u,0x02300278u,0x00c80058u,0x00c002a0u,0x01e80290u,0x00e00058u,0x00d802a0u,0x02180290u,0x00c80198u,0x00c002c0u,0x01e802b0u,0x00e00198u,0x00d802c0u,0x021802b0u,0x00f00000u,0x00f00000u, \
   0x031800f8u,0x03180220u,0x032801e0u,0x034800f8u,0x03480220u,0x041001e0u,0x03780158u,0x03780088u,0x038801e0u,0x04700158u,0x04700088u,0x03b801e0u,0x02a00230u,0x02a00228u,0x01e80240u,0x02300230u,0x02300228u,0x02180240u,0x01c00200u,0x01c00078u,0x00c80040u,0x02080200u,0x02080078u,0x00e00040u,0x01c00090u,0x01c001a8u,0x00c80208u,0x02080090u,0x020801a8u,0x00e00208u,0x00f00000u,0x00f00000u, \
-  0x032800f8u,0x03280118u,0x02680100u,0x041000f8u,0x04100118u,0x01200100u,0x03880158u,0x03880010u,0x01380160u,0x03b80158u,0x03b80010u,0x01500160u,0x01e80230u,0x01e80288u,0x00c80020u,0x02180230u,0x02180288u,0x00e00020u,0x02a00038u,0x02a00070u,0x00c00068u,0x02300038u,0x02300070u,0x00d80068u,0x02a00098u,0x02a000b0u,0x00c000a8u,0x02300098u,0x023000b0u,0x00d800a8u,0x00f00000u,0x00f00000u, \
-  0x01100120u,0x011000b8u,0x02780250u,0x02480120u,0x024800b8u,0x01180250u,0x01600180u,0x01600018u,0x01300168u,0x01580180u,0x01580018u,0x01280168u,0x00d00060u,0x00d00008u,0x00c00048u,0x00e80060u,0x00e80008u,0x00d80048u,0x01e80038u,0x01e80078u,0x014801c0u,0x02180038u,0x02180078u,0x02e001c0u,0x01e80098u,0x01e801a8u,0x01980110u,0x02180098u,0x021801a8u,0x02d80110u,0x00f00000u,0x00f00000u, \
-  0x031002c8u,0x032002c8u,0x031000b8u,0x034002c8u,0x035002c8u,0x034000b8u,0x037002c8u,0x038002c8u,0x03700018u,0x03a002c8u,0x03b002c8u,0x03a00018u,0x01d00268u,0x01e00268u,0x01d00008u,0x02000268u,0x02100268u,0x02000008u,0x03c001b0u,0x03c001d8u,0x01b001c8u,0x03f001b0u,0x03f001d8u,0x017801c8u,0x04200210u,0x04200170u,0x014002d0u,0x04500210u,0x04500170u,0x01a802d0u,0x00f00000u,0x00f00000u, \
+  0x032800f8u,0x03280118u,0x02680100u,0x041000f8u,0x04100118u,0x01200100u,0x03880158u,0x03880010u,0x01800160u,0x03b80158u,0x03b80010u,0x01500160u,0x02400230u,0x02400288u,0x00c80020u,0x02180230u,0x02180288u,0x00e00020u,0x02a00038u,0x02a00070u,0x00c00068u,0x02300038u,0x02300070u,0x00d80068u,0x02a00098u,0x02a000b0u,0x00c000a8u,0x02300098u,0x023000b0u,0x00d800a8u,0x00f00000u,0x00f00000u, \
+  0x01100120u,0x011000b8u,0x02780250u,0x02480120u,0x024800b8u,0x01180250u,0x01600180u,0x01600018u,0x01300168u,0x01580180u,0x01580018u,0x01280168u,0x00d00060u,0x00d00008u,0x00c00048u,0x00e80060u,0x00e80008u,0x00d80048u,0x02400038u,0x02400078u,0x014801c0u,0x02180038u,0x02180078u,0x02e001c0u,0x02400098u,0x024001a8u,0x02200110u,0x02180098u,0x021801a8u,0x02900110u,0x00f00000u,0x00f00000u, \
+  0x031002c8u,0x032002c8u,0x031000b8u,0x034002c8u,0x035002c8u,0x034000b8u,0x037002c8u,0x038002c8u,0x03700018u,0x049802c8u,0x03b002c8u,0x04980018u,0x01d80268u,0x01e00268u,0x01d80008u,0x02880268u,0x02100268u,0x02000008u,0x03c001b0u,0x03c001d8u,0x01b001c8u,0x048801b0u,0x048801d8u,0x017801c8u,0x04200210u,0x04200170u,0x016802d0u,0x04500210u,0x04500170u,0x01a802d0u,0x00f00000u,0x00f00000u, \
   0x03080250u,0x030800b8u,0x03200250u,0x03380250u,0x033800b8u,0x03500250u,0x03680168u,0x03680018u,0x03800168u,0x03980168u,0x03980018u,0x03b00168u,0x01c80048u,0x01c80008u,0x01e00048u,0x01f80048u,0x01f80008u,0x02100048u,0x03d801b8u,0x03d802d8u,0x01d001d0u,0x040801b8u,0x040802d8u,0x020001d0u,0x04380218u,0x043800e8u,0x01d00270u,0x04680218u,0x046800e8u,0x02000270u,0x00f00000u,0x00f00000u, \
   0x00f00000u,0x00f00000u,0x00f00000u,0x00f00000u,0x00f00000u,0x00f00000u,0x00f00000u,0x00f00000u,0x00f00000u,0x00f00000u,0x00f00000u,0x00f00000u,0x00f00000u,0x00f00000u,0x00f00000u,0x00f00000u,0x00f00000u,0x00f00000u,0x03e801b8u,0x03e801d8u,0x01e00068u,0x041801b8u,0x041801d8u,0x02100068u,0x04480218u,0x04480170u,0x01e000a8u,0x04780218u,0x04780170u,0x021000a8u,0x00f00000u,0x00f00000u, \
   0x00f00000u,0x00f00000u,0x00f00000u,0x00f00000u,0x00f00000u,0x00f00000u,0x00f00000u,0x00f00000u,0x00f00000u,0x00f00000u,0x00f00000u,0x00f00000u,0x00f00000u,0x00f00000u,0x00f00000u,0x00f00000u,0x00f00000u,0x00f00000u,0x00d00148u,0x00d001d0u,0x03a80238u,0x00e80148u,0x00e801d0u,0x04000238u,0x00d000c0u,0x00d00270u,0x04300260u,0x00e800c0u,0x00e80270u,0x04600260u,0x00f00000u,0x00f00000u, \
@@ -80,15 +80,15 @@
   0x00f00000u,0x00f00000u,0x00f00000u,0x00f00000u,0x00f00000u,0x00f00000u,0x00f00000u,0x00f00000u,0x00f00000u,0x00f00000u,0x00f00000u,0x00f00000u,0x00f00000u,0x00f00000u,0x00f00000u,0x00f00000u,0x00f00000u,0x00f00000u,0x01d00058u,0x01e00058u,0x00f00000u,0x02000058u,0x02100058u,0x00f00000u,0x01d00198u,0x01e00198u,0x00f00000u,0x02000198u,0x02100198u,0x00f00000u,0x00f00000u,0x00f00000u, \
   0x00f00000u,0x00f00000u,0x00f00000u,0x00f00000u,0x00f00000u,0x00f00000u,0x00f00000u,0x00f00000u,0x00f00000u,0x00f00000u,0x00f00000u,0x00f00000u,0x00f00000u,0x00f00000u,0x00f00000u,0x00f00000u,0x00f00000u,0x00f00000u,0x01c80068u,0x01c801d0u,0x00f00000u,0x01f80068u,0x01f801d0u,0x00f00000u,0x01c800a8u,0x01c80270u,0x00f00000u,0x01f800a8u,0x01f80270u,0x00f00000u,0x00f00000u,0x00f00000u, \
   0x00f00000u,0x00f00000u,0x00f00000u,0x00f00000u,0x00f00000u,0x00f00000u,0x00f00000u,0x00f00000u,0x00f00000u,0x00f00000u,0x00f00000u,0x00f00000u,0x00f00000u,0x00f00000u,0x00f00000u,0x00f00000u,0x00f00000u,0x00f00000u,0x03c801c8u,0x03c80238u,0x00f00000u,0x03f801c8u,0x03f80238u,0x00f00000u,0x042802d0u,0x04280260u,0x00f00000u,0x045802d0u,0x04580260u,0x00f00000u,0x00f00000u,0x00f00000u, \
-  0x00180128u,0x00180130u,0x02680100u,0x00300138u,0x00300140u,0x01200100u,0x00200188u,0x00200190u,0x01380160u,0x00380198u,0x003801a0u,0x01500160u,0x001000c8u,0x001000d0u,0x00f00270u,0x002800d8u,0x002800e0u,0x00f00270u,0x004000c8u,0x004000d0u,0x00f00290u,0x004800d8u,0x004800e0u,0x00f00290u,0x00500128u,0x00500130u,0x00f00220u,0x00580138u,0x00580140u,0x00f00220u,0x00f00000u,0x00f00000u, \
+  0x00180128u,0x00180130u,0x02680100u,0x00300138u,0x00300140u,0x02500100u,0x00200188u,0x00200190u,0x01800160u,0x00380198u,0x003801a0u,0x01080160u,0x001000c8u,0x001000d0u,0x00f00270u,0x002800d8u,0x002800e0u,0x00f00270u,0x004000c8u,0x004000d0u,0x00f00290u,0x004800d8u,0x004800e0u,0x00f00290u,0x00500128u,0x00500130u,0x00f00220u,0x00580138u,0x00580140u,0x00f00220u,0x00f00000u,0x00f00000u, \
   0x000000f0u,0x00000110u,0x02780108u,0x000000f0u,0x00000110u,0x01180108u,0x00080150u,0x00080080u,0x01300168u,0x00080150u,0x00080080u,0x01280168u,0x00f00010u,0x00f00050u,0x01c00278u,0x00f00010u,0x00f00050u,0x02080278u,0x00f00030u,0x00f00070u,0x01c00298u,0x00f00030u,0x00f00070u,0x02080298u,0x00f00090u,0x00f00028u,0x01c002b8u,0x00f00090u,0x00f00028u,0x020802b8u,0x00f00000u,0x00f00000u, \
-  0x030000f0u,0x03000118u,0x031000e8u,0x03d000f0u,0x03d00118u,0x034000e8u,0x03600150u,0x03600178u,0x03700148u,0x03900150u,0x03900178u,0x03a00148u,0x00c80268u,0x00c00280u,0x02a00278u,0x00e00268u,0x00d80280u,0x02300278u,0x006001b0u,0x006001d0u,0x02a00298u,0x006001b0u,0x006001d0u,0x02300298u,0x00780210u,0x00780230u,0x02a002b8u,0x00780210u,0x00780230u,0x023002b8u,0x00f00000u,0x00f00000u, \
+  0x030000f0u,0x03000118u,0x04a800e8u,0x03d000f0u,0x03d00118u,0x04b000e8u,0x04d80150u,0x04d80178u,0x03700148u,0x03900150u,0x03900178u,0x04980148u,0x00c80268u,0x00c00280u,0x02a00278u,0x00e00268u,0x00d80280u,0x02300278u,0x006002c8u,0x006001d0u,0x02a00298u,0x006002c8u,0x006001d0u,0x02300298u,0x00780210u,0x00780230u,0x02a002b8u,0x00780210u,0x00780230u,0x023002b8u,0x00f002e0u,0x00f002e0u, \
   0x031800f8u,0x03180110u,0x03200108u,0x034800f8u,0x03480110u,0x03500108u,0x03780158u,0x03780080u,0x03800168u,0x04700158u,0x04700080u,0x03b00168u,0x01c00010u,0x01c00058u,0x01e80270u,0x02080010u,0x02080058u,0x02180270u,0x006801e8u,0x006801f0u,0x01e80290u,0x007001f8u,0x00700200u,0x02180290u,0x00800248u,0x00800250u,0x01e80220u,0x00880258u,0x00880260u,0x02180220u,0x00f00000u,0x00f00000u, \
   0x032800f8u,0x03280118u,0x00f00000u,0x041000f8u,0x04100118u,0x00f00000u,0x03880158u,0x03880178u,0x00f00000u,0x03b80158u,0x03b80178u,0x00f00000u,0x02a00018u,0x02a00050u,0x00c80020u,0x02300018u,0x02300050u,0x00e00020u,0x00c80288u,0x00c002a0u,0x00c80040u,0x00e00288u,0x00d802a0u,0x00e00040u,0x00c802a8u,0x00c002c0u,0x00c801a8u,0x00e002a8u,0x00d802c0u,0x00e001a8u,0x00f00000u,0x00f00000u, \
-  0x01100120u,0x011000e8u,0x00f00000u,0x02480120u,0x024800e8u,0x00f00000u,0x01600180u,0x01600148u,0x00f00000u,0x01580180u,0x01580148u,0x00f00000u,0x01e80018u,0x01e80058u,0x00c00048u,0x02180018u,0x02180058u,0x00d80048u,0x01c00030u,0x01c00078u,0x00c00068u,0x02080030u,0x02080078u,0x00d80068u,0x01c00090u,0x01c000b8u,0x00c000a8u,0x02080090u,0x020800b8u,0x00d800a8u,0x00f00000u,0x00f00000u, \
-  0x03080108u,0x030800e8u,0x00f00000u,0x03380108u,0x033800e8u,0x00f00000u,0x03680168u,0x03680148u,0x00f00000u,0x03980168u,0x03980148u,0x00f00000u,0x00d00060u,0x00d00008u,0x01d00008u,0x00e80060u,0x00e80008u,0x02000008u,0x02a00038u,0x02a00070u,0x014801c0u,0x02300038u,0x02300070u,0x02e001c0u,0x02a00098u,0x02a00028u,0x019802b0u,0x02300098u,0x02300028u,0x02d802b0u,0x00f00000u,0x00f00000u, \
-  0x00f00000u,0x00f00000u,0x00f00000u,0x00f00000u,0x00f00000u,0x00f00000u,0x00f00000u,0x00f00000u,0x00f00000u,0x00f00000u,0x00f00000u,0x00f00000u,0x01d00268u,0x01e00268u,0x01e00048u,0x02000268u,0x02100268u,0x02100048u,0x01e80038u,0x01e80078u,0x01b001c8u,0x02180038u,0x02180078u,0x017801c8u,0x01e80098u,0x01e800b8u,0x01400228u,0x02180098u,0x021800b8u,0x01a80228u,0x00f00000u,0x00f00000u, \
-  0x00f00000u,0x00f00000u,0x00f00000u,0x00f00000u,0x00f00000u,0x00f00000u,0x00f00000u,0x00f00000u,0x00f00000u,0x00f00000u,0x00f00000u,0x00f00000u,0x01c80048u,0x01c80008u,0x00f00000u,0x01f80048u,0x01f80008u,0x00f00000u,0x03c001b0u,0x03c001d8u,0x01d00238u,0x03f001b0u,0x03f001d8u,0x02000238u,0x04200210u,0x042000a0u,0x01d00170u,0x04500210u,0x045000a0u,0x02000170u,0x00f00000u,0x00f00000u, \
+  0x01100120u,0x011000e8u,0x00f002e0u,0x02480120u,0x024800e8u,0x00f002e0u,0x01600180u,0x01600148u,0x00f002e0u,0x01580180u,0x01580148u,0x00f002e0u,0x01e80018u,0x01e80058u,0x00c002d0u,0x02180018u,0x02180058u,0x00d80048u,0x01000030u,0x01000078u,0x00c00068u,0x02080030u,0x02080078u,0x00d80068u,0x01000090u,0x010000b8u,0x00c000a8u,0x02080090u,0x020800b8u,0x00d800a8u,0x00f00000u,0x00f00000u, \
+  0x03080108u,0x030802f8u,0x00f00000u,0x03380108u,0x033802f8u,0x00f00000u,0x04800168u,0x04800148u,0x00f00000u,0x03980168u,0x03980148u,0x00f00000u,0x00d00060u,0x00d002f0u,0x01d802f0u,0x00e80060u,0x00e80008u,0x02000008u,0x02a00038u,0x02a00070u,0x014801c0u,0x02300038u,0x02300070u,0x02e001c0u,0x02a00098u,0x02a00028u,0x019802b0u,0x02300098u,0x02300028u,0x02d802b0u,0x00f00000u,0x00f00000u, \
+  0x00f00000u,0x00f00000u,0x00f00000u,0x00f00000u,0x00f00000u,0x00f00000u,0x00f00000u,0x00f00000u,0x00f00000u,0x00f00000u,0x00f00000u,0x00f00000u,0x01d00268u,0x01e00268u,0x01e00048u,0x02000268u,0x02100268u,0x021002d0u,0x01e802d8u,0x01e80078u,0x01b001c8u,0x021802d8u,0x02180078u,0x017801c8u,0x01e80098u,0x01e800b8u,0x01400228u,0x02180098u,0x021800b8u,0x01a80228u,0x00f00000u,0x00f00000u, \
+  0x00f00000u,0x00f00000u,0x00f00000u,0x00f00000u,0x00f00000u,0x00f00000u,0x00f00000u,0x00f00000u,0x00f00000u,0x00f00000u,0x00f00000u,0x00f00000u,0x01c80048u,0x01c80008u,0x00f00000u,0x01f80048u,0x01f80008u,0x00f00000u,0x03c001b0u,0x03c001d8u,0x01d80238u,0x048801b0u,0x048801d8u,0x02000238u,0x04200210u,0x042000a0u,0x01d80170u,0x04500210u,0x045000a0u,0x02000170u,0x00f00000u,0x00f00000u, \
   0x00f00000u,0x00f00000u,0x00f00000u,0x00f00000u,0x00f00000u,0x00f00000u,0x00f00000u,0x00f00000u,0x00f00000u,0x00f00000u,0x00f00000u,0x00f00000u,0x00f00000u,0x00f00000u,0x00f00000u,0x00f00000u,0x00f00000u,0x00f00000u,0x03d801b8u,0x03d801d0u,0x01e00068u,0x040801b8u,0x040801d0u,0x02100068u,0x04380218u,0x04380230u,0x01e000a8u,0x04680218u,0x04680230u,0x021000a8u,0x00f00000u,0x00f00000u, \
   0x00f00000u,0x00f00000u,0x00f00000u,0x00f00000u,0x00f00000u,0x00f00000u,0x00f00000u,0x00f00000u,0x00f00000u,0x00f00000u,0x00f00000u,0x00f00000u,0x00f00000u,0x00f00000u,0x00f00000u,0x00f00000u,0x00f00000u,0x00f00000u,0x03e801b8u,0x03e801d8u,0x03a800b0u,0x041801b8u,0x041801d8u,0x040000b0u,0x04480218u,0x044800a0u,0x04300208u,0x04780218u,0x047800a0u,0x04600208u,0x00f00000u,0x00f00000u, \
   0x00f00000u,0x00f00000u,0x00f00000u,0x00f00000u,0x00f00000u,0x00f00000u,0x00f00000u,0x00f00000u,0x00f00000u,0x00f00000u,0x00f00000u,0x00f00000u,0x00f00000u,0x00f00000u,0x00f00000u,0x00f00000u,0x00f00000u,0x00f00000u,0x00d00088u,0x00d00238u,0x03e001c8u,0x00e80088u,0x00e80238u,0x035801c8u,0x00d000c0u,0x00d00170u,0x04400228u,0x00e800c0u,0x00e80170u,0x03300228u,0x00f00000u,0x00f00000u, \
diff --git a/trifocal_pose_estimation_using_improved_gpuhc_b200/csrc/hc_problem_gen_coupled_quadrics_8x8.h b/trifocal_pose_estimation_using_improved_gpuhc_b200/csrc/hc_problem_gen_coupled_quadrics_8x8.h
--- a/trifocal_pose_estimation_using_improved_gpuhc_b200/csrc/hc_problem_gen_coupled_quadrics_8x8.h
+++ b/trifocal_pose_estimation_using_improved_gpuhc_b200/csrc/hc_problem_gen_coupled_quadrics_8x8.h
@@ -31,7 +31,7 @@
 #define HCG_TBL_INIT { \
   0x0008a050u,0x00040000u,0x00041008u,0x00042010u,0x00043018u,0x00044020u,0x00045028u,0x00046030u,0x00047038u,0x000c9040u,0x000ca040u,0x000ca048u,0x000ca050u,0x0010a050u,0x0008a050u,0x0008a050u,0x0008a050u,0x0008a050u,0x0008a050u,0x0008a050u,0x0008a050u,0x0008a050u,0x0008a050u,0x0008a050u,0x0008a050u,0x0008a050u,0x0008a050u,0x0008a050u,0x0008a050u,0x0008a050u,0x0008a050u,0x0008a050u, \
   0x0008a050u,0x00040000u,0x00041008u,0x00042010u,0x00043018u,0x00044020u,0x00045028u,0x00046030u,0x00047038u,0x000c9040u,0x000ca040u,0x000ca048u,0x0008a050u,0x0008a050u,0x0008a050u,0x0008a050u,0x0008a050u,0x0008a050u,0x0008a050u,0x0008a050u,0x0008a050u,0x0008a050u,0x0008a050u,0x0008a050u,0x0008a050u,0x0008a050u,0x0008a050u,0x0008a050u,0x0008a050u,0x0008a050u,0x0008a050u,0x0008a050u, \
-  0x00400000u,0x00401000u,0x00400808u,0x00404040u,0x00401008u,0x00401010u,0x00401810u,0x00402010u,0x00401818u,0x00402818u,0x00402020u,0x00403020u,0x00402828u,0x00403028u,0x00403828u,0x00400030u,0x00403030u,0x00403830u,0x00400838u,0x00403838u,0x00404040u,0x00404040u,0x00404040u,0x00404040u,0x00404040u,0x00404040u,0x00401808u,0x00404040u,0x00404040u,0x00404040u,0x00404040u,0x00404040u, \
+  0x00400000u,0x00401000u,0x00400808u,0x00404040u,0x00401008u,0x00401010u,0x00401810u,0x00402010u,0x00401818u,0x00402818u,0x00402020u,0x00403020u,0x00402828u,0x00403028u,0x00403828u,0x00400030u,0x00403030u,0x00403830u,0x00400838u,0x00403838u,0x00400000u,0x00404040u,0x00401818u,0x00404040u,0x00404040u,0x00404040u,0x00401808u,0x00404040u,0x00404040u,0x00404040u,0x00404040u,0x00404040u, \
   0x00181008u,0x00383028u,0x00404040u,0x00404040u,0x00404040u,0x00404040u,0x00404040u,0x00404040u,0x00404040u,0x00404040u,0x00404040u,0x00404040u,0x00404040u,0x00404040u,0x00404040u,0x00404040u,0x00404040u,0x00404040u,0x00404040u,0x00404040u,0x00404040u,0x00404040u,0x00404040u,0x00404040u,0x00404040u,0x00404040u,0x00404040u,0x00404040u,0x00404040u,0x00404040u,0x00404040u,0x00404040u, \
   0x00000068u,0x00100050u,0x00200068u,0x00300050u,0x00400058u,0x00100050u,0x00400058u,0x00300050u,0x00400000u,0x00400000u,0x00400000u,0x00400000u,0x00400000u,0x00400000u,0x00400000u,0x00400000u,0x00400000u,0x00400000u,0x00400000u,0x00400000u,0x00400000u,0x00400000u,0x00400000u,0x00400000u,0x00400000u,0x00400000u,0x00400000u,0x00400000u,0x00400000u,0x00400000u,0x00400000u,0x00400000u, \
   0x00180050u,0x00080068u,0x01300048u,0x00400000u,0x00380050u,0x00400058u,0x00400000u,0x00400000u,0x00400000u,0x00400000u,0x00400000u,0x00400000u,0x00400000u,0x00400000u,0x00400000u,0x00400000u,0x00400000u,0x00400000u,0x00400000u,0x00400000u,0x00400000u,0x00400000u,0x00400000u,0x00400000u,0x00400000u,0x00400000u,0x00400000u,0x00400000u,0x00400000u,0x00400000u,0x00400000u,0x00400000u, \
@@ -40,7 +40,7 @@
   0x01880048u,0x00400000u,0x00380050u,0x00280068u,0x00400000u,0x00400000u,0x00180050u,0x00400058u,0x00400000u,0x00400000u,0x00400000u,0x00400000u,0x00400000u,0x00400000u,0x00400000u,0x00400000u,0x00400000u,0x00400000u,0x00400000u,0x00400000u,0x00400000u,0x00400000u,0x00400000u,0x00400000u,0x00400000u,0x00400000u,0x00400000u,0x00400000u,0x00400000u,0x00400000u,0x00400000u,0x00400000u, \
   0x01700048u,0x00400000u,0x00400058u,0x00000050u,0x00300068u,0x00400000u,0x00400000u,0x00200050u,0x00400000u,0x00400000u,0x00400000u,0x00400000u,0x00400000u,0x00400000u,0x00400000u,0x00400000u,0x00400000u,0x00400000u,0x00400000u,0x00400000u,0x00400000u,0x00400000u,0x00400000u,0x00400000u,0x00400000u,0x00400000u,0x00400000u,0x00400000u,0x00400000u,0x00400000u,0x00400000u,0x00400000u, \
   0x01680048u,0x00400000u,0x00280050u,0x00400058u,0x00080050u,0x00380068u,0x00400000u,0x00400000u,0x00400000u,0x00400000u,0x00400000u,0x00400000u,0x00400000u,0x00400000u,0x00400000u,0x00400000u,0x00400000u,0x00400000u,0x00400000u,0x00400000u,0x00400000u,0x00400000u,0x00400000u,0x00400000u,0x00400000u,0x00400000u,0x00400000u,0x00400000u,0x00400000u,0x00400000u,0x00400000u,0x00400000u, \
-  0x01000060u,0x01100060u,0x01500060u,0x01600060u,0x01800060u,0x01980060u,0x01280060u,0x01400060u,0x00400000u,0x00400000u,0x00400000u,0x00400000u,0x00400000u,0x00400000u,0x00400000u,0x00400000u,0x00400000u,0x00400000u,0x00400000u,0x00400000u,0x00400000u,0x00400000u,0x00400000u,0x00400000u,0x00400000u,0x00400000u,0x00400000u,0x00400000u,0x00400000u,0x00400000u,0x00400000u,0x00400000u, \
+  0x01a00060u,0x01100060u,0x01500060u,0x01600060u,0x01800060u,0x01980060u,0x01280060u,0x01b00060u,0x00400000u,0x00400000u,0x00400000u,0x00400000u,0x00400000u,0x00400000u,0x00400000u,0x00400000u,0x00400000u,0x00400000u,0x00400000u,0x00400000u,0x00400000u,0x00400000u,0x00400000u,0x00400000u,0x00400000u,0x00400000u,0x00400000u,0x00400000u,0x00400000u,0x00400000u,0x00400000u,0x00400000u, \
   0x00400008u,0x00400010u,0x00400028u,0x00400030u,0x00400038u,0x00400040u,0x00400018u,0x00400020u,0x00400000u,0x00400000u,0x00400000u,0x00400000u,0x00400000u,0x00400000u,0x00400000u,0x00400000u,0x00400000u,0x00400000u,0x00400000u,0x00400000u,0x00400000u,0x00400000u,0x00400000u,0x00400000u,0x00400000u,0x00400000u,0x00400000u,0x00400000u,0x00400000u,0x00400000u,0x00400000u,0x00400000u, \
   0x01d00050u,0x01380050u,0x01700050u,0x01780050u,0x01900050u,0x01080050u,0x01480050u,0x01580050u,0x00400000u,0x00400000u,0x00400000u,0x00400000u,0x00400000u,0x00400000u,0x00400000u,0x00400000u,0x00400000u,0x00400000u,0x00400000u,0x00400000u,0x00400000u,0x00400000u,0x00400000u,0x00400000u,0x00400000u,0x00400000u,0x00400000u,0x00400000u,0x00400000u,0x00400000u,0x00400000u,0x00400000u, \
   0x00100058u,0x00180058u,0x00300058u,0x00380058u,0x00000058u,0x00080058u,0x00200058u,0x00280058u,0x00400000u,0x00400000u,0x00400000u,0x00400000u,0x00400000u,0x00400000u,0x00400000u,0x00400000u,0x00400000u,0x00400000u,0x00400000u,0x00400000u,0x00400000u,0x00400000u,0x00400000u,0x00400000u,0x00400000u,0x00400000u,0x00400000u,0x00400000u,0x00400000u,0x00400000u,0x00400000u,0x00400000u, \
diff --git a/trifocal_pose_estimation_using_improved_gpuhc_b200/csrc/hc_problem_gen_mixed_12x12.h b/trifocal_pose_estimation_using_improved_gpuhc_b200/csrc/hc_problem_gen_mixed_12x12.h
--- a/trifocal_pose_estimation_using_improved_gpuhc_b200/csrc/hc_problem_gen_mixed_12x12.h
+++ b/trifocal_pose_estimation_using_improved_gpuhc_b200/csrc/hc_problem_gen_mixed_12x12.h
@@ -2,7 +2,7 @@
 #define HC_PROBLEM_GEN_H
 #define HCG_N 12
 #define HCG_NUM_PARAMS 14
-#define HCG_NUM_CQ 17
+#define HCG_NUM_CQ 20
 #define HCG_NUM_DQ 15
 #define HCG_CQ_ROUNDS 1
 #define HCG_DQ_ROUNDS 1
@@ -31,13 +31,13 @@
 #define HCG_TBL_INIT { \
   0x0008e070u,0x00040000u,0x00041008u,0x0010e070u,0x00043018u,0x00044020u,0x00045028u,0x0004e030u,0x0004e038u,0x0004e040u,0x0004e048u,0x0004e050u,0x0004e058u,0x000ce060u,0x000ce068u,0x000ce070u,0x00042010u,0x0008e070u,0x0008e070u,0x0008e070u,0x0008e070u,0x0008e070u,0x0008e070u,0x0008e070u,0x0008e070u,0x0008e070u,0x0008e070u,0x0008e070u,0x0008e070u,0x0008e070u,0x0008e070u,0x0008e070u, \
   0x0008e070u,0x00040000u,0x00041008u,0x00042010u,0x00043018u,0x00044020u,0x00045028u,0x0004e030u,0x0004e038u,0x0004e040u,0x0004e048u,0x0004e050u,0x0004e058u,0x000ce060u,0x000ce068u,0x0008e070u,0x0008e070u,0x0008e070u,0x0008e070u,0x0008e070u,0x0008e070u,0x0008e070u,0x0008e070u,0x0008e070u,0x0008e070u,0x0008e070u,0x0008e070u,0x0008e070u,0x0008e070u,0x0008e070u,0x0008e070u,0x0008e070u, \
-  0x00600000u,0x00602800u,0x00603800u,0x00600808u,0x00603008u,0x00604008u,0x00601010u,0x00603810u,0x00604810u,0x00605830u,0x00604018u,0x00605018u,0x00602020u,0x00604820u,0x00605820u,0x00602828u,0x00605028u,0x00601818u,0x00606060u,0x00606060u,0x00606060u,0x00606060u,0x00606060u,0x00606060u,0x00606060u,0x00606060u,0x00606060u,0x00606060u,0x00606060u,0x00606060u,0x00606060u,0x00606060u, \
+  0x00600000u,0x00602800u,0x00603800u,0x00600808u,0x00603008u,0x00604008u,0x00601010u,0x00603810u,0x00604810u,0x00605830u,0x00604018u,0x00605018u,0x00602020u,0x00604820u,0x00605820u,0x00602828u,0x00605028u,0x00601818u,0x00601010u,0x00606060u,0x00602020u,0x00606060u,0x00606060u,0x00606060u,0x00606060u,0x00606060u,0x00606060u,0x00606060u,0x00606060u,0x00606060u,0x00606060u,0x00606060u, \
   0x00000018u,0x00380068u,0x00100018u,0x00380070u,0x00600000u,0x00280070u,0x00480068u,0x00200018u,0x00600000u,0x00480070u,0x00600000u,0x00580070u,0x00600000u,0x00600000u,0x00600000u,0x00600000u,0x00600000u,0x00600000u,0x00600000u,0x00600000u,0x00600000u,0x00600000u,0x00600000u,0x00600000u,0x00600000u,0x00600000u,0x00600000u,0x00600000u,0x00600000u,0x00600000u,0x00600000u,0x00600000u, \
   0x00300068u,0x00080018u,0x00400068u,0x00600000u,0x00400070u,0x00000070u,0x00180018u,0x00500068u,0x00280018u,0x00600000u,0x00500070u,0x00600000u,0x00600000u,0x00600000u,0x00600000u,0x00600000u,0x00600000u,0x00600000u,0x00600000u,0x00600000u,0x00600000u,0x00600000u,0x00600000u,0x00600000u,0x00600000u,0x00600000u,0x00600000u,0x00600000u,0x00600000u,0x00600000u,0x00600000u,0x00600000u, \
   0x00080068u,0x00600000u,0x00180068u,0x00600078u,0x00080070u,0x00600000u,0x00600000u,0x00280068u,0x00580068u,0x00600078u,0x00180070u,0x00600078u,0x00600000u,0x00600000u,0x00600000u,0x00600000u,0x00600000u,0x00600000u,0x00600000u,0x00600000u,0x00600000u,0x00600000u,0x00600000u,0x00600000u,0x00600000u,0x00600000u,0x00600000u,0x00600000u,0x00600000u,0x00600000u,0x00600000u,0x00600000u, \
   0x00600000u,0x00100068u,0x00600000u,0x00000070u,0x00600078u,0x00600078u,0x00200068u,0x00600000u,0x00300068u,0x00100070u,0x00600078u,0x00200070u,0x00600000u,0x00600000u,0x00600000u,0x00600000u,0x00600000u,0x00600000u,0x00600000u,0x00600000u,0x00600000u,0x00600000u,0x00600000u,0x00600000u,0x00600000u,0x00600000u,0x00600000u,0x00600000u,0x00600000u,0x00600000u,0x00600000u,0x00600000u, \
-  0x01000078u,0x01180078u,0x01300078u,0x00300078u,0x00380078u,0x00580078u,0x01880078u,0x01600078u,0x01780078u,0x00400078u,0x00480078u,0x00500078u,0x00600000u,0x00600000u,0x00600000u,0x00600000u,0x00600000u,0x00600000u,0x00600000u,0x00600000u,0x00600000u,0x00600000u,0x00600000u,0x00600000u,0x00600000u,0x00600000u,0x00600000u,0x00600000u,0x00600000u,0x00600000u,0x00600000u,0x00600000u, \
-  0x00600008u,0x00600010u,0x00600080u,0x00600038u,0x00600040u,0x00600060u,0x00600020u,0x00600028u,0x00600030u,0x00600048u,0x00600050u,0x00600058u,0x00600000u,0x00600000u,0x00600000u,0x00600000u,0x00600000u,0x00600000u,0x00600000u,0x00600000u,0x00600000u,0x00600000u,0x00600000u,0x00600000u,0x00600000u,0x00600000u,0x00600000u,0x00600000u,0x00600000u,0x00600000u,0x00600000u,0x00600000u, \
+  0x01000078u,0x01180078u,0x01900078u,0x00300078u,0x00380078u,0x00580078u,0x01880078u,0x01a00078u,0x01780078u,0x00400078u,0x00480078u,0x00500078u,0x00600000u,0x00600000u,0x00600000u,0x00600000u,0x00600000u,0x00600000u,0x00600000u,0x00600000u,0x00600000u,0x00600000u,0x00600000u,0x00600000u,0x00600000u,0x00600000u,0x00600000u,0x00600000u,0x00600000u,0x00600000u,0x00600000u,0x00600000u, \
+  0x00600008u,0x00600010u,0x00600080u,0x00600038u,0x00600040u,0x00600060u,0x00600020u,0x00600028u,0x00600030u,0x00600048u,0x00600050u,0x00600058u,0x00600098u,0x00600098u,0x00600098u,0x00600098u,0x00600000u,0x00600000u,0x00600000u,0x00600000u,0x00600000u,0x00600000u,0x00600000u,0x00600000u,0x00600000u,0x00600000u,0x00600000u,0x00600000u,0x00600000u,0x00600000u,0x00600000u,0x00600000u, \
   0x01200068u,0x01380068u,0x01500068u,0x01100070u,0x01280070u,0x01080070u,0x01680068u,0x01800068u,0x01480068u,0x01400070u,0x01580070u,0x01700070u,0x00600000u,0x00600000u,0x00600000u,0x00600000u,0x00600000u,0x00600000u,0x00600000u,0x00600000u,0x00600000u,0x00600000u,0x00600000u,0x00600000u,0x00600000u,0x00600000u,0x00600000u,0x00600000u,0x00600000u,0x00600000u,0x00600000u,0x00600000u, \
   0x00600008u,0x00600010u,0x00600018u,0x00600038u,0x00600040u,0x00600060u,0x00600020u,0x00600028u,0x00600030u,0x00600048u,0x00600050u,0x00600058u,0x00600000u,0x00600000u,0x00600000u,0x00600000u,0x00600000u,0x00600000u,0x00600000u,0x00600000u,0x00600000u,0x00600000u,0x00600000u,0x00600000u,0x00600000u,0x00600000u,0x00600000u,0x00600000u,0x00600000u,0x00600000u,0x00600000u,0x00600000u, \
   0x01200068u,0x01380068u,0x01500068u,0x01100070u,0x01280070u,0x01080070u,0x01680068u,0x01800068u,0x01480068u,0x01400070u,0x01580070u,0x01700070u,0x00600000u,0x00600000u,0x00600000u,0x00600000u,0x00600000u,0x00600000u,0x00600000u,0x00600000u,0x00600000u,0x00600000u,0x00600000u,0x00600000u,0x00600000u,0x00600000u,0x00600000u,0x00600000u,0x00600000u,0x00600000u,0x00600000u,0x00600000u, \
```

Measured after the change: 4666 (median of 6 runs). About the same (+0.5%).
